# ryogrid/anime-illust-image-searcher

Hardware: AMD Instinct MI355X
Metric: images/sec tagged (ViT fwd) (higher is better)
Workload: dtype f16; 1 GPU; wd-tagger ViT-B/16 448px 16-bit-operand forward + sigmoid + MCut tag selection, batch 64 per GPU, u8 NHWC images resident in HBM (BASELINE.json configs[1]); batch_per_gpu=64, image=448x448x3 u8, classes=10861, parallelism=single GPU

## Files before the change

### anime-illust-image-searcher_amd/csrc/gemm.hip

```cpp
#include <atomic>
#include <cstdlib>
#include <type_traits>

#include "vit_internal.h"

namespace hipts {
namespace {

#ifndef HIPTS_DW_SNAKE
#define HIPTS_DW_SNAKE 1
#endif
#if HIPTS_DW_SNAKE
#define HIPTS_SNAKE_J(i, j) (((i) & 1) ? 3 - (j) : (j))
#else
#define HIPTS_SNAKE_J(i, j) (j)
#endif
#ifndef HIPTS_MFMA_ORDER
#define HIPTS_MFMA_ORDER 1
#endif
#include "gemm_epi.h"


template <int EPI>
__global__ __launch_bounds__(512) void gemm_kernel(const GemmArgs a, int tiles_m, int tiles_n) {
    extern __shared__ __attribute__((aligned(16))) char smem[];
    const int tid = threadIdx.x, lane = tid & 63, wave = tid >> 6;
    const int wave_m = wave >> 2, wave_n = wave & 3;

    const int nwg = tiles_m * tiles_n;
    int bid = blockIdx.x;
    {
        const int q = nwg >> 3, r = nwg & 7, xcd = bid & 7, loc = bid >> 3;
        bid = (xcd < r ? xcd * (q + 1) : r * (q + 1) + (xcd - r) * q) + loc;
    }
    const int tm = bid / tiles_n, tn = bid % tiles_n;
    const int m0 = tm * BM, n0 = tn * BN;
    const int K = a.K, nt = K / BK;
    const int w_rows = tiles_n * BN;

    f32x4 acc[8][4];
#pragma unroll
    for (int i = 0; i < 8; ++i)
#pragma unroll
        for (int j = 0; j < 4; ++j) acc[i][j] = f32x4{0.f, 0.f, 0.f, 0.f};

    stage_tile(a.A, a.M, K, m0, 0, smem, wave, lane);
    stage_tile(a.W, w_rows, K, n0, 0, smem + TILE_BYTES, wave, lane);
    asm volatile("s_waitcnt vmcnt(0)" ::: "memory");
    __syncthreads();

    for (int t = 0; t < nt; ++t) {
        char* cur = smem + (t & 1) * STAGE_BYTES;
        if (t + 1 < nt) {
            char* nxt = smem + ((t + 1) & 1) * STAGE_BYTES;
            stage_tile(a.A, a.M, K, m0, t + 1, nxt, wave, lane);
            stage_tile(a.W, w_rows, K, n0, t + 1, nxt + TILE_BYTES, wave, lane);
        }
#pragma unroll
        for (int kk = 0; kk < 2; ++kk) {
            bf16x8 af[8], wf[4];
#pragma unroll
            for (int j = 0; j < 4; ++j) wf[j] = read_frag(cur + TILE_BYTES, wave_n * 4 + j, kk, lane);
#pragma unroll
            for (int i = 0; i < 8; ++i) af[i] = read_frag(cur, wave_m * 8 + i, kk, lane);
#pragma unroll
            for (int i = 0; i < 8; ++i)
#pragma unroll
                for (int j = 0; j < 4; ++j) {
                    if constexpr (EPI == EPI_VT)
                        acc[i][j] = __builtin_amdgcn_mfma_f32_16x16x32_bf16(af[i], wf[j], acc[i][j], 0, 0, 0);
                    else
                        acc[i][j] = __builtin_amdgcn_mfma_f32_16x16x32_bf16(wf[j], af[i], acc[i][j], 0, 0, 0);
                }
        }
        asm volatile("s_waitcnt vmcnt(0)" ::: "memory");
        __syncthreads();
    }

    gemm_epilogue<EPI>(a, acc, m0, n0, wave_m, wave_n, lane);
}

__device__ __forceinline__ void wait_vmcnt(int n) {
    switch (n) {
        case 0: asm volatile("s_waitcnt vmcnt(0)" ::: "memory"); break;
        case 1: asm volatile("s_waitcnt vmcnt(1)" ::: "memory"); break;
        case 2: asm volatile("s_waitcnt vmcnt(2)" ::: "memory"); break;
        case 3: asm volatile("s_waitcnt vmcnt(3)" ::: "memory"); break;
        case 4: asm volatile("s_waitcnt vmcnt(4)" ::: "memory"); break;
        case 5: asm volatile("s_waitcnt vmcnt(5)" ::: "memory"); break;
        case 6: asm volatile("s_waitcnt vmcnt(6)" ::: "memory"); break;
        case 7: asm volatile("s_waitcnt vmcnt(7)" ::: "memory"); break;
        default: asm volatile("s_waitcnt vmcnt(8)" ::: "memory"); break;
    }
}

template <int EPI, int MR = 8, bool F16 = false, bool OP8 = false, bool SK = false, bool INT = false>
__global__ __launch_bounds__(512) __attribute__((amdgpu_num_vgpr(HIPTS_INT_DEPTH == 3 ? 256 : 240))) void gemm_pp_kernel(const GemmArgs a, int tiles_m, int tiles_n) {
    static_assert(!INT || (EPI == EPI_RESID_XG && MR == 8 && !OP8 && !SK), "INT: the residual epilogue's interior form");
    static_assert(!OP8 || (F16 && MR == 8), "e4m3 operands: half 16-bit outputs, full tiles");
    static_assert(!SK || (!OP8 && MR == 8), "split-K: 16-bit operands, full tiles");
    constexpr int TBM = 2 * MR * 16;
    extern __shared__ __attribute__((aligned(16))) char smem[];
    __shared__ float2 st_table[256];
    __shared__ float2 sw_red[EPI == EPI_SWIGLU ? 1024 : 1];
    __shared__ unsigned sk_ticket[SK ? 4 : 1];
    __shared__ f32x4 colvec[INT ? (EPI == EPI_RESID_XGI ? 768 : 512) : 1];
    const int tid = threadIdx.x, lane = tid & 63;
    const int wave = __builtin_amdgcn_readfirstlane(tid >> 6);
    const int wave_m = wave >> 2, wave_n = wave & 3;

    const int nwg = tiles_m * tiles_n;
    auto tile_origin = [&](int id, int& m0, int& n0) {
        const int q = nwg >> 3, r = nwg & 7, xcd = id & 7, loc = id >> 3;
        const int bid = (xcd < r ? xcd * (q + 1) : r * (q + 1) + (xcd - r) * q) + loc;
        if (a.raster_gn > 0) {
            const int per = tiles_m * a.raster_gn, grp = bid / per, rem = bid - grp * per;
            const int left = tiles_n - grp * a.raster_gn, gn = left < a.raster_gn ? left : a.raster_gn;
            m0 = (rem / gn) * TBM;
            n0 = (grp * a.raster_gn + rem % gn) * BN;
            return;
        }
        if (a.raster_gm > 0) {
            const int per = a.raster_gm * tiles_n, grp = bid / per, rem = bid - grp * per;
            const int left = tiles_m - grp * a.raster_gm, gm = left < a.raster_gm ? left : a.raster_gm;
            m0 = (grp * a.raster_gm + rem % gm) * TBM;
            n0 = (rem / gm) * BN;
            return;
        }
        m0 = (bid / tiles_n) * TBM;
        n0 = (bid % tiles_n) * BN;
    };
    const int K = OP8 ? a.K / 2 : a.K, nt_all = K / BK;
    const int w_rows = tiles_n * BN;
    const int S = SK ? a.sk_slices : 1;
    const int n_items = SK ? a.sk_first + (nwg - a.sk_first) * S : nwg;
    auto decode = [&](int item, int& tid_, int& slice_, int& kt0_, int& ntl_) {
        if (!SK || item < a.sk_first) {
            tid_ = item; slice_ = -1; kt0_ = 0; ntl_ = nt_all;
        } else {
            const int j = item - a.sk_first;
            tid_ = a.sk_first + j / S;
            slice_ = j - (j / S) * S;
            kt0_ = slice_ * nt_all / S;
            ntl_ = (slice_ + 1) * nt_all / S - kt0_;
        }
    };
    const int scale_w = (127 - a.w_exp) * 0x01010101, scale_1 = 127 * 0x01010101;

    int stamp_tile = 0;
#define PPSTAMP(idx)                                                                                     \
    do {                                                                                                 \
        if (a.stamps && blockIdx.x == 8 && stamp_tile < 8) {                                             \
            __builtin_amdgcn_sched_barrier(0);                                                           \
            const unsigned long long ts_ = __builtin_readcyclecounter();                                 \
            if (lane == 0) a.stamps[wave * 64 + stamp_tile * 8 + (idx)] = ts_;                           \
            __builtin_amdgcn_sched_barrier(0);                                                           \
        }                                                                                                \
    } while (0)
    int tile = blockIdx.x, m0, n0;
    int tix, slice, kt0, nt;
    decode(tile, tix, slice, kt0, nt);
    tile_origin(tix, m0, n0);
    int par = 0;

    if (wave * 4 < 4 * MR) stage_tile(a.A, a.M, K, m0, kt0, smem, wave, lane);
    stage_tile(a.W, w_rows, K, n0, kt0, smem + TILE_BYTES, wave, lane);
    if constexpr (INT) {
        for (int i = tid; i < (a.N >> 2); i += 512) {
            colvec[i] = reinterpret_cast<const f32x4*>(a.ln_gamma)[i];
            colvec[256 + i] = reinterpret_cast<const f32x4*>(a.bias)[i];
            if constexpr (EPI == EPI_RESID_XGI) colvec[512 + i] = reinterpret_cast<const f32x4*>(a.col_u)[i];
        }
        asm volatile("s_waitcnt lgkmcnt(0)" ::: "memory");
    }

    for (;;) {
        f32x4 acc[MR][4];
#pragma unroll
        for (int i = 0; i < MR; ++i)
#pragma unroll
            for (int j = 0; j < 4; ++j) acc[i][j] = f32x4{0.f, 0.f, 0.f, 0.f};

        const bf16_t* src[8];
        int dst[8];
        {
            const int row_in = lane >> 3;
            const int chunk = (lane & 7) ^ row_in;
            auto slot = [&](int idx, bool isW, int rb8) {
                int grow = (isW ? n0 : m0) + rb8 * 8 + row_in;
                const int lim = isW ? w_rows : a.M;
                grow = grow < lim ? grow : lim - 1;
                src[idx] = (isW ? a.W : a.A) + (size_t)grow * K + (size_t)(kt0 + 1) * BK + chunk * 8;
                dst[idx] = (isW ? TILE_BYTES : 0) + rb8 * 1024;
            };
            for (int u = 0; u < 2; ++u) {
                const int e = 2 * wave + u;
                slot(0 + u, true, e);
                slot(2 + u, true, 16 + e);
                slot(4 + u, false, e < 8 ? e : 2 * MR + (e - 8));
            }
            if constexpr (MR == 8) {
                for (int u = 0; u < 2; ++u) {
                    const int e = 2 * wave + u;
                    slot(6 + u, false, e < 8 ? 8 + e : 2 * MR + 8 + (e - 8));
                }
            } else if constexpr (MR == 6) {
                slot(6, false, wave < 4 ? 8 + wave : 2 * MR + 8 + (wave - 4));
                src[7] = src[6];
                dst[7] = dst[6];
            } else {
                static_assert(MR == 7, "tile heights: 256, 224 or 192 rows");
                auto hi = [](int f) { return f < 6 ? 8 + f : 2 * MR + 8 + (f - 6); };
                if (wave < 4) {
                    slot(6, false, hi(2 * wave));
                    slot(7, false, hi(2 * wave + 1));
                } else {
                    slot(6, false, hi(8 + (wave - 4)));
                    src[7] = src[6];
                    dst[7] = dst[6];
                }
            }
        }
        const int n_hi = (MR == 8 || (MR == 7 && wave < 4)) ? 2 : 1;
        PPSTAMP(0);
        asm volatile("s_waitcnt vmcnt(0)" ::: "memory");
        PPSTAMP(1);
        __builtin_amdgcn_s_barrier();
        if (wave_m == 1) __builtin_amdgcn_s_barrier();
        PPSTAMP(2);
        if (a.stamps && blockIdx.x == 8 && stamp_tile < 8 && lane == 0) a.stamps[wave * 64 + stamp_tile * 8 + 6] = wall_clock64();
        if (HIPTS_STAGE_AHEAD && !HIPTS_STAGE_ORDER_OLD && nt > 1) {
            char* st1 = smem + ((par + 1) & 1) * STAGE_BYTES;
            for (int k : {4, 5, 0, 1}) {
                glds16(src[k], st1 + dst[k]);
                src[k] += BK;
            }
        }

        bf16x8 wf[2][4];
        i32x8 wf8[4], af8[4];
        unsigned xpf = 0;
        for (int t = 0; t < nt; ++t) {
            const char* cur = smem + ((par + t) & 1) * STAGE_BYTES;
            char* nxt = smem + ((par + t + 1) & 1) * STAGE_BYTES;
            const bool more = t + 1 < nt;
#pragma unroll
            for (int p = 0; p < 4; ++p) {
                const int mh = p >> 1, kk = p & 1;
                bf16x8 af[4];
                if constexpr (OP8) {
                    if (p < 2) {
#pragma unroll
                        for (int jj = 0; jj < 2; ++jj) wf8[2 * kk + jj] = read_frag8(cur + TILE_BYTES, wave_n * 4 + 2 * kk + jj, lane);
                    }
                    if (kk == 0) {
#pragma unroll
                        for (int i = 0; i < 4; ++i) af8[i] = read_frag8(cur, wave_m * MR + mh * 4 + i, lane);
                    }
                } else {
                if (p < 2) {
#pragma unroll
                    for (int j = 0; j < 4; ++j) wf[kk][j] = read_frag(cur + TILE_BYTES, wave_n * 4 + j, kk, lane);
                }
#pragma unroll
                for (int i = 0; i < 4; ++i)
                    if (mh * 4 + i < MR) af[i] = read_frag(cur, wave_m * MR + mh * 4 + i, kk, lane);
                }
                if (more) {
                    auto issue = [&](int k) {
                        glds16(src[k], nxt + dst[k]);
                        src[k] += BK;
                    };
                    if (HIPTS_STAGE_ORDER_OLD) {
                        issue(2 * p);
                        if (p < 3 || n_hi == 2) issue(2 * p + 1);
                        if (p == 3) {
                            if (n_hi == 2) asm volatile("s_waitcnt vmcnt(2)" ::: "memory");
                            else asm volatile("s_waitcnt vmcnt(1)" ::: "memory");
                        } else if (p == 1) {
                            asm volatile("s_waitcnt vmcnt(4)" ::: "memory");
                        }
                    } else if (HIPTS_STAGE_AHEAD) {
                        if (p == 0) {
                            issue(2); issue(3);
                        } else if (p == 1) {
                            issue(6);
                            if (n_hi == 2) issue(7);
                            wait_vmcnt(6 + n_hi);
                        } else if (p == 3) {
                            if (t + 2 < nt) {
                                for (int k : {4, 5, 0, 1}) {
                                    glds16(src[k], const_cast<char*>(cur) + dst[k]);
                                    src[k] += BK;
                                }
                                wait_vmcnt(n_hi + 4);
                            } else {
                                wait_vmcnt(n_hi);
                            }
                        }
                    } else {
                        if (p == 0) {
                            issue(4); issue(5); issue(0); issue(1);
                            if (HIPTS_STAGE_W_EARLY) { issue(2); issue(3); }
                        } else if (p == 1) {
                            if (!HIPTS_STAGE_W_EARLY) { issue(2); issue(3); }
                            asm volatile("s_waitcnt vmcnt(6)" ::: "memory");
                        } else if (p == 2) {
                            issue(6);
                            if (n_hi == 2) issue(7);
                        } else {
                            if (n_hi == 2) asm volatile("s_waitcnt vmcnt(2)" ::: "memory");
                            else asm volatile("s_waitcnt vmcnt(1)" ::: "memory");
                        }
                    }
                } else if (p == 1) {
                    asm volatile("s_waitcnt vmcnt(0)" ::: "memory");
                }
                if constexpr (INT) {
                    if (!more && p == 2 && a.epi_prefetch) {
                        const int ldx = a.ld_out ? a.ld_out : a.N;
                        const char* xb = reinterpret_cast<const char*>(a.out_f32 + (size_t)(m0 + wave_m * 128) * ldx + n0 + wave_n * 64);
                        const unsigned o0 = (unsigned)(((lane >> 1) * ldx + (lane & 1) * 32) * 4), ost = (unsigned)(32 * ldx * 4);
                        asm volatile("global_load_dword %0, %1, %5\n\tglobal_load_dword %0, %2, %5\n\tglobal_load_dword %0, %3, %5\n\tglobal_load_dword %0, %4, %5"
                                     : "=&v"(xpf)
                                     : "v"(o0), "v"(o0 + ost), "v"(o0 + 2 * ost), "v"(o0 + 3 * ost), "s"(xb)
                                     : "memory");
                    }
                }
                __builtin_amdgcn_sched_barrier(0);
                __builtin_amdgcn_s_barrier();
                __builtin_amdgcn_sched_barrier(0);
                asm volatile("s_waitcnt lgkmcnt(0)" ::: "memory");
                __builtin_amdgcn_sched_barrier(0);
                __builtin_amdgcn_s_setprio(1);
                if constexpr (OP8) {
#pragma unroll
                    for (int i = 0; i < 4; ++i)
#pragma unroll
                        for (int jj = 0; jj < 2; ++jj) {
                            const int j = 2 * kk + jj;
                            if constexpr (EPI == EPI_VT)
                                acc[mh * 4 + i][j] = mfma_16x16x128_e4m3(af8[i], wf8[j], acc[mh * 4 + i][j], scale_1, scale_w);
                            else
                                acc[mh * 4 + i][j] = mfma_16x16x128_e4m3(wf8[j], af8[i], acc[mh * 4 + i][j], scale_w, scale_1);
                        }
                } else {
#pragma unroll
                for (int ij = 0; ij < 16; ++ij) {
#if HIPTS_MFMA_ORDER == 2
                    const int j = ij >> 2, i = ij & 3;
#elif HIPTS_MFMA_ORDER == 1
                    const int i = ij >> 2, j = (i & 1) ? 3 - (ij & 3) : (ij & 3);
#else
                    const int i = ij >> 2, j = ij & 3;
#endif
                    if (mh * 4 + i >= MR) continue;
                    if constexpr (EPI == EPI_VT)
                        acc[mh * 4 + i][j] = mfma_16x16x32<F16>(af[i], wf[kk][j], acc[mh * 4 + i][j]);
                    else
                        acc[mh * 4 + i][j] = mfma_16x16x32<F16>(wf[kk][j], af[i], acc[mh * 4 + i][j]);
                }
                }
                __builtin_amdgcn_s_setprio(0);
                __builtin_amdgcn_sched_barrier(0);
                __builtin_amdgcn_s_barrier();
                __builtin_amdgcn_sched_barrier(0);
            }
        }
        if (wave_m == 0) __builtin_amdgcn_s_barrier();
        PPSTAMP(3);
        if (a.stamps && blockIdx.x == 8 && stamp_tile < 8 && lane == 0) a.stamps[wave * 64 + stamp_tile * 8 + 7] = wall_clock64();

        f32x4 bias_pre[4];
        if constexpr (INT) {
#pragma unroll
            for (int j = 0; j < 4; ++j) bias_pre[j] = f32x4{0.f, 0.f, 0.f, 0.f};
        } else {
            load_bias<EPI>(a, n0, wave_n, lane, bias_pre);
        }
        constexpr bool FOLDABLE = EPI == EPI_VT || EPI == EPI_GELU || EPI == EPI_STAR || EPI == EPI_QK || EPI == EPI_QK_ROPE || EPI == EPI_SWIGLU ||
                                  EPI == EPI_RESID_ROWSTAT || EPI == EPI_RESID_XGI;
        const bool fold_st = FOLDABLE && a.stat_in != nullptr;
        const bool fold_many = fold_st && a.stat_in_blocks > 4;
        float2 st_pv[4];
        if (fold_st && !fold_many && tid < TBM) row_stat_request(a, m0 + tid, st_pv);
        const int next = tile + gridDim.x;
        const bool has_next = next < n_items;
        int m0n = 0, n0n = 0, tixn = 0, slicen = -1, kt0n = 0, ntn = nt_all;
        const int par_next = (par + nt) & 1;
        if (has_next) {
            decode(next, tixn, slicen, kt0n, ntn);
            tile_origin(tixn, m0n, n0n);
            char* st = smem + par_next * STAGE_BYTES;
            if (wave * 4 < 4 * MR) stage_tile(a.A, a.M, K, m0n, kt0n, st, wave, lane);
            stage_tile(a.W, w_rows, K, n0n, kt0n, st + TILE_BYTES, wave, lane);
        }
        PPSTAMP(4);
        bool run_epilogue = true;
        if constexpr (SK) {
            if (slice >= 0) {
                constexpr size_t SLAB = (size_t)TBM * BN * 4;
                const int tl = tix - a.sk_first;
                unsigned* tickets = reinterpret_cast<unsigned*>(a.sk_ws);
                char* slabs = reinterpret_cast<char*>(a.sk_ws) + 4096 + (size_t)tl * S * SLAB;
                {
                    const auto rs = __builtin_amdgcn_make_buffer_rsrc(slabs + (size_t)slice * SLAB, 0, (int)SLAB, 0x00020000);
                    typedef unsigned int u32x4 __attribute__((ext_vector_type(4)));
#pragma unroll
                    for (int i = 0; i < MR; ++i)
#pragma unroll
                        for (int j = 0; j < 4; ++j)
                            __builtin_amdgcn_raw_buffer_store_b128(__builtin_bit_cast(u32x4, acc[i][j]), rs, (((wave * MR + i) * 4 + j) * 64 + lane) * 16, 0, 16);
                }
                asm volatile("s_waitcnt vmcnt(0)" ::: "memory");
                __builtin_amdgcn_s_barrier();
                if (threadIdx.x == 0)
                    sk_ticket[0] = __hip_atomic_fetch_add(tickets + tl, 1u, __ATOMIC_RELAXED, __HIP_MEMORY_SCOPE_AGENT);
                __builtin_amdgcn_fence(__ATOMIC_RELEASE, "workgroup");
                __builtin_amdgcn_s_barrier();
                __builtin_amdgcn_fence(__ATOMIC_ACQUIRE, "workgroup");
                const unsigned ticket = sk_ticket[0];
                if (ticket != (unsigned)(S - 1)) {
                    run_epilogue = false;
                } else {
                    if (threadIdx.x == 0) {
                        __builtin_amdgcn_fence(__ATOMIC_ACQUIRE, "agent");
                        __hip_atomic_store(tickets + tl, 0u, __ATOMIC_RELAXED, __HIP_MEMORY_SCOPE_AGENT);
                    }
                    asm volatile("s_waitcnt vmcnt(0)" ::: "memory");
                    __builtin_amdgcn_s_barrier();
                    const f32x4* sl = reinterpret_cast<const f32x4*>(slabs) + (size_t)(wave * MR * 4) * 64 + lane;
#pragma unroll
                    for (int i = 0; i < MR; ++i) {
#pragma unroll
                        for (int j = 0; j < 4; ++j) acc[i][j] = sl[(size_t)(i * 4 + j) * 64];
                        for (int sx = 1; sx < S; ++sx) {
                            const f32x4* sp = sl + (size_t)sx * (SLAB / 16);
                            f32x4 v[4];
#pragma unroll
                            for (int j = 0; j < 4; ++j) v[j] = sp[(size_t)(i * 4 + j) * 64];
#pragma unroll
                            for (int j = 0; j < 4; ++j) acc[i][j] = acc[i][j] + v[j];
                        }
                    }
                }
            }
        }
        if (run_epilogue) {
        if (fold_st) {
            if (fold_many) {
                if (tid < TBM) st_table[tid] = row_stat(a, m0 + tid);
            } else if (tid < TBM) st_table[tid] = row_stat_finish(a, st_pv);
            __builtin_amdgcn_fence(__ATOMIC_RELEASE, "workgroup");
            __builtin_amdgcn_s_barrier();
            __builtin_amdgcn_fence(__ATOMIC_ACQUIRE, "workgroup");
        }
        bool staged = false;
        if constexpr (EPI == EPI_VT || EPI == EPI_GELU || EPI == EPI_STAR || EPI == EPI_QK || EPI == EPI_QK_ROPE || EPI == EPI_SWIGLU) {
            const bool ok = EPI == EPI_VT                            ? (a.tokens % 8 == 0 && a.tokens_pad % 8 == 0)
                            : (EPI == EPI_QK || EPI == EPI_QK_ROPE) ? (a.dim % 64 == 0)
                                                                     : ((a.ld_out ? a.ld_out : a.N) % 8 == 0);
            if (ok) {
                float2* red = (EPI == EPI_SWIGLU && a.stat_part) ? sw_red : nullptr;
                gemm_epilogue_staged<EPI, MR, F16>(a, acc, m0, n0, wave_m, wave_n, lane,
                                                   smem + ((par + nt + 1) & 1) * STAGE_BYTES + wave * 8192, bias_pre, fold_st ? st_table : nullptr, red);
                staged = true;
                if constexpr (EPI == EPI_SWIGLU) {
                    if (red) {
                        __builtin_amdgcn_fence(__ATOMIC_RELEASE, "workgroup");
                        __builtin_amdgcn_s_barrier();
                        __builtin_amdgcn_fence(__ATOMIC_ACQUIRE, "workgroup");
                        if (tid < TBM) {
                            const float2 p0 = red[tid * 4], p1 = red[tid * 4 + 1], p2 = red[tid * 4 + 2], p3 = red[tid * 4 + 3];
                            const int m = m0 + tid;
                            if (m < a.M)
                                *reinterpret_cast<float2*>(a.stat_part + 2 * ((size_t)(n0 >> 8) * a.stat_stride + m)) =
                                    make_float2((p0.x + p1.x) + (p2.x + p3.x), (p0.y + p1.y) + (p2.y + p3.y));
                        }
                    }
                }
            }
        }
        if (!staged)
            gemm_epilogue<EPI, MR, F16, INT>(a, acc, m0, n0, wave_m, wave_n, lane, bias_pre, smem + ((par + nt + 1) & 1) * STAGE_BYTES,
                                             fold_st ? st_table : nullptr, INT ? colvec : nullptr);
        }
        if (a.epi_prio) __builtin_amdgcn_s_setprio(0);
        if constexpr (INT) asm volatile("" ::"v"(xpf));
        PPSTAMP(5);
        ++stamp_tile;
        if (!has_next) break;
        tile = next;
        tix = tixn;
        slice = slicen;
        kt0 = kt0n;
        nt = ntn;
        m0 = m0n;
        n0 = n0n;
        par = par_next;
    }
}

#define PP2_STAMP(idx)                                                                                   \
    if constexpr (STAMP) {                                                                               \
        if (blockIdx.x == 0 && (t == 10 || t == 11)) {                                                   \
            __builtin_amdgcn_sched_barrier(0);                                                           \
            unsigned long long ts_;                                                                      \
            asm volatile("s_memtime %0\n\ts_waitcnt lgkmcnt(0)" : "=s"(ts_)::"memory");                 \
            if (lane == 0) a.stamps[wave * 64 + (t - 10) * 16 + mh * 8 + (idx)] = ts_;                   \
            __builtin_amdgcn_sched_barrier(0);                                                           \
        }                                                                                                \
    }

template <int EPI, bool STAMP = false>
__global__ __launch_bounds__(512) void gemm_pp2_kernel(const GemmArgs a, int tiles_m, int tiles_n) {
    extern __shared__ __attribute__((aligned(16))) char smem[];
    const int tid = threadIdx.x, lane = tid & 63;
    const int wave = __builtin_amdgcn_readfirstlane(tid >> 6);
    const int wave_m = wave >> 2, wave_n = wave & 3;

    const int nwg = tiles_m * tiles_n;
    int bid = blockIdx.x;
    {
        const int q = nwg >> 3, r = nwg & 7, xcd = bid & 7, loc = bid >> 3;
        bid = (xcd < r ? xcd * (q + 1) : r * (q + 1) + (xcd - r) * q) + loc;
    }
    const int tm = bid / tiles_n, tn = bid % tiles_n;
    const int m0 = tm * BM, n0 = tn * BN;
    const int K = a.K, nt = K / BK;
    const int w_rows = tiles_n * BN;

    f32x4 acc[8][4];
#pragma unroll
    for (int i = 0; i < 8; ++i)
#pragma unroll
        for (int j = 0; j < 4; ++j) acc[i][j] = f32x4{0.f, 0.f, 0.f, 0.f};

    stage_tile(a.A, a.M, K, m0, 0, smem, wave, lane);
    stage_tile(a.W, w_rows, K, n0, 0, smem + TILE_BYTES, wave, lane);

    const bf16_t* src[8];
    int dst[8];
    {
        const int row_in = lane >> 3;
        const int chunk = (lane & 7) ^ row_in;
        auto slot = [&](int idx, bool isW, int rb8) {
            int grow = (isW ? n0 : m0) + rb8 * 8 + row_in;
            const int lim = isW ? w_rows : a.M;
            grow = grow < lim ? grow : lim - 1;
            src[idx] = (isW ? a.W : a.A) + (size_t)grow * K + BK + chunk * 8;
            dst[idx] = (isW ? TILE_BYTES : 0) + rb8 * 1024;
        };
        for (int u = 0; u < 4; ++u) slot(u, true, 4 * wave + u);
        for (int u = 0; u < 2; ++u) {
            const int e = 2 * wave + u;
            slot(4 + u, false, e < 8 ? e : e + 8);
            slot(6 + u, false, e < 8 ? 8 + e : 16 + e);
        }
    }
    asm volatile("s_waitcnt vmcnt(0)" ::: "memory");
    __builtin_amdgcn_s_barrier();
    if (wave_m == 1) __builtin_amdgcn_s_barrier();

    bf16x8 wf[2][4];
    for (int t = 0; t < nt; ++t) {
        const char* cur = smem + (t & 1) * STAGE_BYTES;
        char* nxt = smem + ((t + 1) & 1) * STAGE_BYTES;
        const bool more = t + 1 < nt;
#pragma unroll
        for (int mh = 0; mh < 2; ++mh) {
            PP2_STAMP(0)
            bf16x8 af[2][4];
            if (mh == 0) {
#pragma unroll
                for (int kk = 0; kk < 2; ++kk)
#pragma unroll
                    for (int j = 0; j < 4; ++j) wf[kk][j] = read_frag(cur + TILE_BYTES, wave_n * 4 + j, kk, lane);
            }
#pragma unroll
            for (int kk = 0; kk < 2; ++kk)
#pragma unroll
                for (int i = 0; i < 4; ++i) af[kk][i] = read_frag(cur, wave_m * 8 + mh * 4 + i, kk, lane);
            if (more) {
                if (mh == 0) {
#pragma unroll
                    for (int u = 0; u < 6; ++u) {
                        glds16(src[u], nxt + dst[u]);
                        src[u] += BK;
                    }
                    PP2_STAMP(1)
                    asm volatile("s_waitcnt vmcnt(6)" ::: "memory");
                } else {
#pragma unroll
                    for (int u = 6; u < 8; ++u) {
                        glds16(src[u], nxt + dst[u]);
                        src[u] += BK;
                    }
                    PP2_STAMP(1)
                    asm volatile("s_waitcnt vmcnt(2)" ::: "memory");
                }
            } else if (mh == 0) {
                asm volatile("s_waitcnt vmcnt(0)" ::: "memory");
            }
            PP2_STAMP(2)
            __builtin_amdgcn_sched_barrier(0);
            __builtin_amdgcn_s_barrier();
            __builtin_amdgcn_sched_barrier(0);
            PP2_STAMP(3)
            asm volatile("s_waitcnt lgkmcnt(0)" ::: "memory");
            __builtin_amdgcn_sched_barrier(0);
            PP2_STAMP(4)
            __builtin_amdgcn_s_setprio(1);
#pragma unroll
            for (int kk = 0; kk < 2; ++kk)
#pragma unroll
                for (int i = 0; i < 4; ++i)
#pragma unroll
                    for (int j = 0; j < 4; ++j) {
                        if constexpr (EPI == EPI_VT)
                            acc[mh * 4 + i][j] = __builtin_amdgcn_mfma_f32_16x16x32_bf16(af[kk][i], wf[kk][j], acc[mh * 4 + i][j], 0, 0, 0);
                        else
                            acc[mh * 4 + i][j] = __builtin_amdgcn_mfma_f32_16x16x32_bf16(wf[kk][j], af[kk][i], acc[mh * 4 + i][j], 0, 0, 0);
                    }
            __builtin_amdgcn_s_setprio(0);
            PP2_STAMP(5)
            __builtin_amdgcn_sched_barrier(0);
            __builtin_amdgcn_s_barrier();
            __builtin_amdgcn_sched_barrier(0);
            PP2_STAMP(6)
        }
    }
    if (wave_m == 0) __builtin_amdgcn_s_barrier();
    gemm_epilogue<EPI>(a, acc, m0, n0, wave_m, wave_n, lane);
}

constexpr int S3_BN = 128, S3_BK = 32, S3_STAGE = (BM + S3_BN) * S3_BK * 2, S3_LDS = 3 * S3_STAGE;

__device__ __forceinline__ void s3_stage(const GemmArgs& a, int m0, int n0, int w_rows, int kt, char* st, int wave, int lane) {
    const int row_in = lane >> 2;
    const int chunk = (lane & 3) ^ (((row_in >> 3) & 1) << 1);
    const size_t koff = (size_t)kt * S3_BK + chunk * 8;
#pragma unroll
    for (int i = 0; i < 4; ++i) {
        const int rb = wave * 4 + i;
        int grow = m0 + rb * 16 + row_in;
        grow = grow < a.M ? grow : a.M - 1;
        glds16(a.A + (size_t)grow * a.K + koff, st + rb * 1024);
    }
#pragma unroll
    for (int i = 0; i < 2; ++i) {
        const int rb = wave * 2 + i;
        int grow = n0 + rb * 16 + row_in;
        grow = grow < w_rows ? grow : w_rows - 1;
        glds16(a.W + (size_t)grow * a.K + koff, st + BM * S3_BK * 2 + rb * 1024);
    }
}

__device__ __forceinline__ bf16x8 s3_frag(const char* base, int rowblk, int lane) {
    const int r = lane & 15;
    const int c = (lane >> 4) ^ (((r >> 3) & 1) << 1);
    return *reinterpret_cast<const bf16x8*>(base + rowblk * 1024 + r * 64 + c * 16);
}

template <int EPI>
__global__ __launch_bounds__(256, 2) void gemm_s3_kernel(const GemmArgs a, int tiles_m, int tiles_n) {
    extern __shared__ __attribute__((aligned(16))) char smem[];
    const int tid = threadIdx.x, lane = tid & 63;
    const int wave = __builtin_amdgcn_readfirstlane(tid >> 6);
    const int wave_m = wave >> 1, wave_n = wave & 1;
    const int nwg = tiles_m * tiles_n;
    int bid = blockIdx.x;
    {
        const int q = nwg >> 3, r = nwg & 7, xcd = bid & 7, loc = bid >> 3;
        bid = (xcd < r ? xcd * (q + 1) : r * (q + 1) + (xcd - r) * q) + loc;
    }
    const int tm = bid / tiles_n, tn = bid % tiles_n;
    const int m0 = tm * BM, n0 = tn * S3_BN;
    const int nt = a.K / S3_BK;
    const int w_rows = ((a.N + 255) / 256) * 256;

    f32x4 acc[8][4];
#pragma unroll
    for (int i = 0; i < 8; ++i)
#pragma unroll
        for (int j = 0; j < 4; ++j) acc[i][j] = f32x4{0.f, 0.f, 0.f, 0.f};

    s3_stage(a, m0, n0, w_rows, 0, smem, wave, lane);
    if (nt > 1) s3_stage(a, m0, n0, w_rows, 1, smem + S3_STAGE, wave, lane);
    int slot = 0;
    for (int t = 0; t < nt; ++t) {
        if (t + 1 < nt) asm volatile("s_waitcnt vmcnt(6)" ::: "memory");
        else asm volatile("s_waitcnt vmcnt(0)" ::: "memory");
        __builtin_amdgcn_s_barrier();
        __builtin_amdgcn_sched_barrier(0);
        if (t + 2 < nt) {
            int s2 = slot + 2;
            s2 = s2 >= 3 ? s2 - 3 : s2;
            s3_stage(a, m0, n0, w_rows, t + 2, smem + s2 * S3_STAGE, wave, lane);
        }
        const char* cur = smem + slot * S3_STAGE;
        bf16x8 af[8], wf[4];
#pragma unroll
        for (int j = 0; j < 4; ++j) wf[j] = s3_frag(cur + BM * S3_BK * 2, wave_n * 4 + j, lane);
#pragma unroll
        for (int i = 0; i < 8; ++i) af[i] = s3_frag(cur, wave_m * 8 + i, lane);
#pragma unroll
        for (int i = 0; i < 8; ++i)
#pragma unroll
            for (int j = 0; j < 4; ++j) {
                if constexpr (EPI == EPI_VT)
                    acc[i][j] = __builtin_amdgcn_mfma_f32_16x16x32_bf16(af[i], wf[j], acc[i][j], 0, 0, 0);
                else
                    acc[i][j] = __builtin_amdgcn_mfma_f32_16x16x32_bf16(wf[j], af[i], acc[i][j], 0, 0, 0);
            }
        slot = slot == 2 ? 0 : slot + 1;
    }
    gemm_epilogue<EPI>(a, acc, m0, n0, wave_m, wave_n, lane);
}

constexpr int DW_BM = 256, DW_BN = 128, DW_BK = 32;
constexpr int DW_A_BYTES = DW_BM * DW_BK * 2;
constexpr int DW_STAGE = (DW_BM + DW_BN) * DW_BK * 2;
constexpr int DW_LDS = 3 * DW_STAGE;

template <int EPI, bool F16>
__global__ __launch_bounds__(256, 2) void gemm_dw_kernel(const GemmArgs a, int tiles_m, int tiles_n) {
    extern __shared__ __attribute__((aligned(16))) char smem[];
    const int tid = threadIdx.x, lane = tid & 63;
    const int wave = __builtin_amdgcn_readfirstlane(tid >> 6);
    const int wave_m = wave >> 1, wave_n = wave & 1;
    const int nwg = tiles_m * tiles_n;
    int bid = blockIdx.x;
    {
        const int q = nwg >> 3, r = nwg & 7, xcd = bid & 7, loc = bid >> 3;
        bid = (xcd < r ? xcd * (q + 1) : r * (q + 1) + (xcd - r) * q) + loc;
    }
    const int tm = bid / tiles_n, tn = bid % tiles_n;
    const int m0 = tm * DW_BM, n0 = tn * DW_BN;
    const int K = a.K, nt = K / DW_BK;
    const int w_rows = ((a.N + 255) / 256) * 256;

    const bf16_t* src[6];
    int dst[6];
    {
        const int r = lane >> 2, q = (lane & 3) ^ ((r >> 2) & 3);
#pragma unroll
        for (int i = 0; i < 4; ++i) {
            const int rb = wave * 4 + i;
            int grow = m0 + rb * 16 + r;
            grow = grow < a.M ? grow : a.M - 1;
            src[i] = a.A + (size_t)grow * K + q * 8;
            dst[i] = rb * 1024;
        }
#pragma unroll
        for (int i = 0; i < 2; ++i) {
            const int rb = wave * 2 + i;
            int grow = n0 + rb * 16 + r;
            grow = grow < w_rows ? grow : w_rows - 1;
            src[4 + i] = a.W + (size_t)grow * K + q * 8;
            dst[4 + i] = DW_A_BYTES + rb * 1024;
        }
    }
    const int frag_off = (lane & 15) * 64 + (((lane >> 4) ^ (((lane & 15) >> 2) & 3)) * 16);
    auto issue = [&](int i, char* st) {
        glds16(src[i], st + dst[i]);
        src[i] += DW_BK;
    };
    auto frag = [&](const char* base, int rb) { return *reinterpret_cast<const bf16x8*>(base + rb * 1024 + frag_off); };

    f32x4 acc[8][4];
#pragma unroll
    for (int i = 0; i < 8; ++i)
#pragma unroll
        for (int j = 0; j < 4; ++j) acc[i][j] = f32x4{0.f, 0.f, 0.f, 0.f};

    const bool trace = a.stamps && a.trace && blockIdx.x < 4096;
    if (trace && tid == 0) {
        a.stamps[blockIdx.x * 8 + 0] = __builtin_amdgcn_s_getreg(63492);
        a.stamps[blockIdx.x * 8 + 1] = __builtin_amdgcn_s_getreg(63508);
        a.stamps[blockIdx.x * 8 + 2] = wall_clock64();
    }
    const int npro = nt < 3 ? nt : 3;
    for (int s0 = 0; s0 < npro; ++s0)
#pragma unroll
        for (int i = 0; i < 6; ++i) issue(i, smem + s0 * DW_STAGE);
    if (npro == 3) asm volatile("s_waitcnt vmcnt(12)" ::: "memory");
    else if (npro == 2) asm volatile("s_waitcnt vmcnt(6)" ::: "memory");
    else asm volatile("s_waitcnt vmcnt(0)" ::: "memory");
    __builtin_amdgcn_s_barrier();
    __builtin_amdgcn_sched_barrier(0);

    bf16x8 wfr[2][4], alo[2][4], ahi[4];
#pragma unroll
    for (int j = 0; j < 4; ++j) wfr[0][j] = frag(smem + DW_A_BYTES, wave_n * 4 + j);
#pragma unroll
    for (int i = 0; i < 4; ++i) alo[0][i] = frag(smem, wave_m * 8 + i);

    int slot = 0;
    unsigned long long wait_cyc = 0, bar_cyc = 0;
    const unsigned long long loop_t0 = a.stamps ? __builtin_readcyclecounter() : 0;
    const unsigned long long wall_t0 = a.stamps ? wall_clock64() : 0;
    auto mm = [&](f32x4& c, const bf16x8& av, const bf16x8& wv) {
        if constexpr (EPI == EPI_VT) c = mfma_16x16x32<F16>(av, wv, c);
        else c = mfma_16x16x32<F16>(wv, av, c);
    };
    auto step = [&](auto H1, auto H2, auto H3, auto U) {
        constexpr bool has1 = decltype(H1)::value, has2 = decltype(H2)::value, has3 = decltype(H3)::value;
        constexpr int u = decltype(U)::value;
        const char* cur = smem + slot * DW_STAGE;
        const int slot1 = slot == 2 ? 0 : slot + 1;
        const char* nx = smem + slot1 * DW_STAGE;
#pragma unroll
        for (int i = 0; i < 4; ++i)
#pragma unroll
            for (int j = 0; j < 4; ++j) {
                mm(acc[i][HIPTS_SNAKE_J(i, j)], alo[u][i], wfr[u][HIPTS_SNAKE_J(i, j)]);
                if (i == 0) ahi[j] = frag(cur, wave_m * 8 + 4 + j);
                __builtin_amdgcn_sched_barrier(0);
            }
        if constexpr (has1) {
            unsigned long long q0 = 0, q1 = 0;
            if (a.stamps) q0 = __builtin_readcyclecounter();
            if constexpr (has2) asm volatile("s_waitcnt vmcnt(6) lgkmcnt(0)" ::: "memory");
            else asm volatile("s_waitcnt vmcnt(0) lgkmcnt(0)" ::: "memory");
            if (a.stamps) q1 = __builtin_readcyclecounter();
            __builtin_amdgcn_s_barrier();
            if (a.stamps) { const unsigned long long q2 = __builtin_readcyclecounter(); wait_cyc += q1 - q0; bar_cyc += q2 - q1; }
        }
        __builtin_amdgcn_sched_barrier(0);
        char* fill = smem + slot * DW_STAGE;
#pragma unroll
        for (int i = 0; i < 4; ++i)
#pragma unroll
            for (int j = 0; j < 4; ++j) {
                mm(acc[4 + i][HIPTS_SNAKE_J(i, j)], ahi[i], wfr[u][HIPTS_SNAKE_J(i, j)]);
                const int idx = i * 4 + j;
                if constexpr (has1) {
                    if (idx < 4) wfr[u ^ 1][idx] = frag(nx + DW_A_BYTES, wave_n * 4 + idx);
                    else if (idx < 8) alo[u ^ 1][idx - 4] = frag(nx, wave_m * 8 + (idx - 4));
                }
                if constexpr (has3) {
                    if (idx >= 8 && idx < 14) issue(idx - 8, fill);
                }
                __builtin_amdgcn_sched_barrier(0);
            }
        slot = slot1;
    };
    using T = std::true_type;
    using F = std::false_type;
    using U0 = std::integral_constant<int, 0>;
    using U1 = std::integral_constant<int, 1>;
    for (int s = 0; s + 6 <= nt; s += 2) {
        step(T{}, T{}, T{}, U0{});
        step(T{}, T{}, T{}, U1{});
    }
    if (nt >= 4) {
        step(T{}, T{}, T{}, U0{});
        step(T{}, T{}, F{}, U1{});
    }
    step(T{}, F{}, F{}, U0{});
    step(F{}, F{}, F{}, U1{});
    if (trace && tid == 0) a.stamps[blockIdx.x * 8 + 3] = wall_clock64();
    if (a.stamps && !trace && blockIdx.x == 8 && lane == 0) {
        a.stamps[wave * 64 + 0] = __builtin_readcyclecounter() - loop_t0;
        a.stamps[wave * 64 + 1] = wait_cyc;
        a.stamps[wave * 64 + 2] = bar_cyc;
        a.stamps[wave * 64 + 3] = wall_clock64() - wall_t0;
    }
    __builtin_amdgcn_s_barrier();
    if constexpr (EPI == EPI_VT || EPI == EPI_GELU || EPI == EPI_STAR || EPI == EPI_QK || EPI == EPI_QK_ROPE || EPI == EPI_SWIGLU) {
        const bool ok = EPI == EPI_VT                            ? (a.tokens % 8 == 0 && a.tokens_pad % 8 == 0)
                        : (EPI == EPI_QK || EPI == EPI_QK_ROPE) ? (a.dim % 64 == 0)
                                                                 : ((a.ld_out ? a.ld_out : a.N) % 8 == 0);
        if (ok) {
            const float2* st_tab = nullptr;
            if (a.stat_in) {
                float2 pv[4];
                row_stat_request(a, m0 + tid, pv);
                float2* tab = reinterpret_cast<float2*>(smem + 4 * 8192 * 2);
                tab[tid] = row_stat_finish(a, pv);
                __builtin_amdgcn_fence(__ATOMIC_RELEASE, "workgroup");
                __builtin_amdgcn_s_barrier();
                __builtin_amdgcn_fence(__ATOMIC_ACQUIRE, "workgroup");
                st_tab = tab;
            }
            gemm_epilogue_staged<EPI, 8, F16>(a, acc, m0, n0, wave_m, wave_n, lane, smem + wave * 8192, nullptr, st_tab);
            if (trace && tid == 0) a.stamps[blockIdx.x * 8 + 4] = wall_clock64();
            return;
        }
    }
    gemm_epilogue<EPI, 8, F16>(a, acc, m0, n0, wave_m, wave_n, lane, nullptr, smem);
    if (trace && tid == 0) a.stamps[blockIdx.x * 8 + 4] = wall_clock64();
}

std::atomic<long long> g_q4_mask{-1};
unsigned gemm_q4_mask() {
    long long v = g_q4_mask.load(std::memory_order_relaxed);
    if (v < 0) {
        v = getenv("HIPTS_GEMM_Q4") ? (long long)(unsigned)strtoul(getenv("HIPTS_GEMM_Q4"), nullptr, 0) : (long long)GEMM_Q4_DEFAULT_MASK;
        g_q4_mask.store(v, std::memory_order_relaxed);
    }
    return (unsigned)v;
}

int gemm_variant() {
    static int v = -1;
    if (v < 0) {
        const char* e = getenv("HIPTS_GEMM");
        v = (e && strcmp(e, "v1") == 0) ? 0 : (e && strcmp(e, "pp2") == 0) ? 3 : (e && strcmp(e, "s3") == 0) ? 2 : (e && strcmp(e, "dw") == 0) ? 4 : 1;
    }
    return v;
}

template <int EPI>
int launch_t(const GemmArgs& a, hipStream_t s) {
    int dev = 0;
    const int cus_dev = current_device_cus(&dev);
    static PerDevice attr;
    {
      std::lock_guard<std::mutex> lk(attr.mu);
      if (!attr.done(dev)) {
        HIPTS_HIP(hipFuncSetAttribute((const void*)gemm_kernel<EPI>, hipFuncAttributeMaxDynamicSharedMemorySize, LDS_BYTES));
        HIPTS_HIP(hipFuncSetAttribute((const void*)gemm_pp_kernel<EPI, 8, false>, hipFuncAttributeMaxDynamicSharedMemorySize, LDS_BYTES));
        HIPTS_HIP(hipFuncSetAttribute((const void*)gemm_pp_kernel<EPI, 7, false>, hipFuncAttributeMaxDynamicSharedMemorySize, LDS_BYTES));
        HIPTS_HIP(hipFuncSetAttribute((const void*)gemm_pp_kernel<EPI, 8, true>, hipFuncAttributeMaxDynamicSharedMemorySize, LDS_BYTES));
        HIPTS_HIP(hipFuncSetAttribute((const void*)gemm_pp_kernel<EPI, 7, true>, hipFuncAttributeMaxDynamicSharedMemorySize, LDS_BYTES));
        HIPTS_HIP(hipFuncSetAttribute((const void*)gemm_pp_kernel<EPI, 6, true>, hipFuncAttributeMaxDynamicSharedMemorySize, LDS_BYTES));
        HIPTS_HIP(hipFuncSetAttribute((const void*)gemm_pp2_kernel<EPI, false>, hipFuncAttributeMaxDynamicSharedMemorySize, LDS_BYTES));
        HIPTS_HIP(hipFuncSetAttribute((const void*)gemm_s3_kernel<EPI>, hipFuncAttributeMaxDynamicSharedMemorySize, S3_LDS));
        HIPTS_HIP(hipFuncSetAttribute((const void*)gemm_dw_kernel<EPI, false>, hipFuncAttributeMaxDynamicSharedMemorySize, DW_LDS));
        HIPTS_HIP(hipFuncSetAttribute((const void*)gemm_dw_kernel<EPI, true>, hipFuncAttributeMaxDynamicSharedMemorySize, DW_LDS));
        attr.mark(dev);
      }
    }
    const int tiles_m = (a.M + BM - 1) / BM;
    if (a.op8) {
        if constexpr (EPI == EPI_STAR || EPI == EPI_RESID || EPI == EPI_RESCALE || EPI == EPI_RESID_LN || EPI == EPI_QK || EPI == EPI_VT ||
                      EPI == EPI_BIAS) {
            static PerDevice attr8;
            {
                std::lock_guard<std::mutex> lk(attr8.mu);
                if (!attr8.done(dev)) {
                    HIPTS_HIP(hipFuncSetAttribute((const void*)gemm_pp_kernel<EPI, 8, true, true>, hipFuncAttributeMaxDynamicSharedMemorySize, LDS_BYTES));
                    attr8.mark(dev);
                }
            }
            const int cus8 = cus_dev;
            const int tiles_n = (a.N + BN - 1) / BN;
            const int ntile = tiles_m * tiles_n;
            const int slots = cus8 >= 8 ? cus8 / 8 * 8 : cus8;
            gemm_pp_kernel<EPI, 8, true, true><<<ntile > slots ? slots : ntile, 512, LDS_BYTES, s>>>(a, tiles_m, tiles_n);
            HIPTS_LAUNCH_CHECK();
            return HIPTS_OK;
        } else {
            return set_error(HIPTS_ERR_INVALID, "gemm: e4m3 operands are not built for epilogue %d", (int)EPI);
        }
    }
    int variant = gemm_variant();
    if (EPI == EPI_QK_ROPE || EPI == EPI_SWIGLU || EPI == EPI_RESID_XG || EPI == EPI_RESID_XGI) variant = 1;
    if (EPI == EPI_RESID_LN) variant = 1;
    if (variant == 1 && EPI != EPI_HEAD && EPI != EPI_RESID_LN && (!getenv("HIPTS_GEMM") || EPI == EPI_QK_ROPE || EPI == EPI_SWIGLU || EPI == EPI_RESID_XG || EPI == EPI_RESID_XGI)) {
        const int cus0 = cus_dev;
        static const bool auto_dw = !(getenv("HIPTS_GEMM_AUTO_DW") && atoi(getenv("HIPTS_GEMM_AUTO_DW")) == 0);
        static const int dw_limit4 = getenv("HIPTS_GEMM_DW_LIMIT") ? atoi(getenv("HIPTS_GEMM_DW_LIMIT")) : 2;
        if (auto_dw && (long)tiles_m * ((a.N + BN - 1) / BN) * 4 <= (long)cus0 * dw_limit4 && a.M > BM && !((EPI == EPI_RESID_XG || EPI == EPI_RESID_XGI || EPI == EPI_SWIGLU) && a.stat_part)) variant = 4;
    }
    {
        static const unsigned dw_mask = getenv("HIPTS_GEMM_DW_MASK") ? (unsigned)strtoul(getenv("HIPTS_GEMM_DW_MASK"), nullptr, 0) : 0u;
#ifdef HIPTS_X_DW_STAT
        if (variant == 1 && ((dw_mask >> (int)EPI) & 1u) && a.M > BM) variant = 4;
#else
        if (variant == 1 && ((dw_mask >> (int)EPI) & 1u) && a.M > BM && !((EPI == EPI_RESID_XG || EPI == EPI_RESID_XGI) && a.stat_part)) variant = 4;
#endif
    }
    HIPTS_REQUIRE(!a.f16 || variant == 1 || variant == 4, "half-precision operands are only built for the pp and dw GEMM loops");
    if (variant == 4) {
        const int tiles_n = (a.N + DW_BN - 1) / DW_BN;
        if (a.f16) gemm_dw_kernel<EPI, true><<<tiles_m * tiles_n, 256, DW_LDS, s>>>(a, tiles_m, tiles_n);
        else gemm_dw_kernel<EPI, false><<<tiles_m * tiles_n, 256, DW_LDS, s>>>(a, tiles_m, tiles_n);
    } else if (variant == 2) {
        const int tiles_n = (a.N + S3_BN - 1) / S3_BN;
        gemm_s3_kernel<EPI><<<tiles_m * tiles_n, 256, S3_LDS, s>>>(a, tiles_m, tiles_n);
    } else {
        const int tiles_n = (a.N + BN - 1) / BN;
        if (variant == 3) {
            if constexpr (EPI == EPI_GELU) {
                if (a.stamps) {
                    HIPTS_HIP(hipFuncSetAttribute((const void*)gemm_pp2_kernel<EPI, true>, hipFuncAttributeMaxDynamicSharedMemorySize, LDS_BYTES));
                    gemm_pp2_kernel<EPI, true><<<tiles_m * tiles_n, 512, LDS_BYTES, s>>>(a, tiles_m, tiles_n);
                    HIPTS_LAUNCH_CHECK();
                    return HIPTS_OK;
                }
            }
            gemm_pp2_kernel<EPI><<<tiles_m * tiles_n, 512, LDS_BYTES, s>>>(a, tiles_m, tiles_n);
        }
        else if (variant == 1) {
            const int cus = cus_dev;
            static const int min_mr = !getenv("HIPTS_GEMM_BM") ? 6 : strcmp(getenv("HIPTS_GEMM_BM"), "256") == 0 ? 8 : strcmp(getenv("HIPTS_GEMM_BM"), "224") == 0 ? 7 : 6;
            auto tiles_of = [&](int mr) { return (a.M + 32 * mr - 1) / (32 * mr); };
            auto cost_of = [&](int mr) { return ((long)tiles_of(mr) * tiles_n + cus - 1) / cus * (32 * mr); };
            int mr = 8;
            static const int mr_shared = getenv("HIPTS_GEMM_MR_SHARED") ? atoi(getenv("HIPTS_GEMM_MR_SHARED")) : -1;
            if (!a.shared_chip || mr_shared == 1 || (mr_shared != 0 && (long)tiles_of(8) * tiles_n < cus)) {
                long best = cost_of(8) * 93;
                for (int c = 7; c >= (a.f16 ? min_mr : (min_mr > 7 ? min_mr : 7)); --c)
                    if (cost_of(c) * 100 < best) {
                        best = cost_of(c) * 100;
                        mr = c;
                    }
            }
            if (EPI == EPI_HEAD && a.sk_ws && getenv("HIPTS_GEMM_SPLITK_HEAD") && atoi(getenv("HIPTS_GEMM_SPLITK_HEAD")) >= 2) mr = 8;
            const int tiles_mr = tiles_of(mr);
            static const bool persist = !(getenv("HIPTS_GEMM_PERSIST") && strcmp(getenv("HIPTS_GEMM_PERSIST"), "0") == 0);
            const int ntile = tiles_mr * tiles_n;
            const int slots = cus >= 8 ? cus / 8 * 8 : cus;
            const int grid = (persist && ntile > slots) ? slots : ntile;
            static const int raster = getenv("HIPTS_GEMM_RASTER") ? atoi(getenv("HIPTS_GEMM_RASTER")) : 8;
            static const int raster_gn = getenv("HIPTS_GEMM_RASTER_GN") ? atoi(getenv("HIPTS_GEMM_RASTER_GN")) : 6;
            GemmArgs ar = a;
            static const int epi_prio = getenv("HIPTS_EPI_PRIO") ? atoi(getenv("HIPTS_EPI_PRIO")) : 0;
            ar.epi_prio = epi_prio;
            static const int epi_prefetch = getenv("HIPTS_EPI_PREFETCH") ? atoi(getenv("HIPTS_EPI_PREFETCH")) : 0;
            ar.epi_prefetch = epi_prefetch;
            ar.raster_gm = (raster > 0 && tiles_n >= 8) ? raster : 0;
            ar.raster_gn = (raster_gn > 0 && tiles_n >= 8 && tiles_n > raster_gn) ? raster_gn : 0;
            {
                const unsigned q4_mask = gemm_q4_mask();
                if (mr == 8 && ((q4_mask >> (int)EPI) & 1u)) {
                    bool handled = false;
                    const int st = launch_gemm_q4((GemmEpilogue)EPI, ar, s, &handled);
                    if (handled) return st;
                }
            }
            static const bool resid_general = getenv("HIPTS_RESID_GENERAL") && atoi(getenv("HIPTS_RESID_GENERAL")) != 0;
            if constexpr (EPI == EPI_RESID || EPI == EPI_RESID_XG || EPI == EPI_RESID_XGI || EPI == EPI_RESID_ROWSTAT || EPI == EPI_HEAD) {
                static const int sk_env = getenv("HIPTS_GEMM_SPLITK") ? atoi(getenv("HIPTS_GEMM_SPLITK")) : 0;
                static const int sk_head = getenv("HIPTS_GEMM_SPLITK_HEAD") ? atoi(getenv("HIPTS_GEMM_SPLITK_HEAD")) : 0;
                const int sk_max = EPI == EPI_HEAD ? (tiles_mr == 1 ? sk_head : 0) : sk_env;
                static const int sk_minkt = getenv("HIPTS_GEMM_SPLITK_MINKT") ? atoi(getenv("HIPTS_GEMM_SPLITK_MINKT")) : 5;
                const int nkt = a.K / BK;
                const int rem = ntile % slots;
                if (a.sk_ws && mr == 8 && sk_max >= 2 && rem > 0 && rem * 2 <= slots && rem <= 1024) {
                    int sl = std::min(sk_max, std::min(slots / rem, nkt / (sk_minkt > 0 ? sk_minkt : 1)));
                    while (sl >= 2 && 4096 + (size_t)rem * sl * ((size_t)BM * BN * 4) > a.sk_ws_bytes) --sl;
                    if (sl >= 2) {
                        static PerDevice attr_sk;
                        {
                            std::lock_guard<std::mutex> lk(attr_sk.mu);
                            if (!attr_sk.done(dev)) {
                                HIPTS_HIP(hipFuncSetAttribute((const void*)gemm_pp_kernel<EPI, 8, false, false, true>, hipFuncAttributeMaxDynamicSharedMemorySize, LDS_BYTES));
                                HIPTS_HIP(hipFuncSetAttribute((const void*)gemm_pp_kernel<EPI, 8, true, false, true>, hipFuncAttributeMaxDynamicSharedMemorySize, LDS_BYTES));
                                attr_sk.mark(dev);
                            }
                        }
                        ar.sk_first = ntile - rem;
                        ar.sk_slices = sl;
                        const int items = ar.sk_first + rem * sl;
                        const int grid_sk = (persist && items > slots) ? slots : items;
                        if (a.f16) gemm_pp_kernel<EPI, 8, true, false, true><<<grid_sk, 512, LDS_BYTES, s>>>(ar, tiles_m, tiles_n);
                        else gemm_pp_kernel<EPI, 8, false, false, true><<<grid_sk, 512, LDS_BYTES, s>>>(ar, tiles_m, tiles_n);
                        HIPTS_LAUNCH_CHECK();
                        return HIPTS_OK;
                    }
                }
            }
            if constexpr (EPI == EPI_RESID_XG) {
                if (mr == 8 && a.M % 256 == 0 && a.N % 256 == 0 && a.N <= 1024 && !a.pos && !a.res_scale && a.out_bf16 && a.stat_part && !resid_general) {
                    static PerDevice attr_int;
                    {
                        std::lock_guard<std::mutex> lk(attr_int.mu);
                        if (!attr_int.done(dev)) {
                            HIPTS_HIP(hipFuncSetAttribute((const void*)gemm_pp_kernel<EPI, 8, false, false, false, true>, hipFuncAttributeMaxDynamicSharedMemorySize, LDS_BYTES));
                            HIPTS_HIP(hipFuncSetAttribute((const void*)gemm_pp_kernel<EPI, 8, true, false, false, true>, hipFuncAttributeMaxDynamicSharedMemorySize, LDS_BYTES));
                            attr_int.mark(dev);
                        }
                    }
                    if (a.f16) gemm_pp_kernel<EPI, 8, true, false, false, true><<<grid, 512, LDS_BYTES, s>>>(ar, tiles_m, tiles_n);
                    else gemm_pp_kernel<EPI, 8, false, false, false, true><<<grid, 512, LDS_BYTES, s>>>(ar, tiles_m, tiles_n);
                    HIPTS_LAUNCH_CHECK();
                    return HIPTS_OK;
                }
            }
            if (a.f16) {
                if (mr == 6) gemm_pp_kernel<EPI, 6, true><<<grid, 512, LDS_BYTES, s>>>(ar, tiles_mr, tiles_n);
                else if (mr == 7) gemm_pp_kernel<EPI, 7, true><<<grid, 512, LDS_BYTES, s>>>(ar, tiles_mr, tiles_n);
                else gemm_pp_kernel<EPI, 8, true><<<grid, 512, LDS_BYTES, s>>>(ar, tiles_m, tiles_n);
            } else {
                if (mr == 7) gemm_pp_kernel<EPI, 7, false><<<grid, 512, LDS_BYTES, s>>>(ar, tiles_mr, tiles_n);
                else gemm_pp_kernel<EPI, 8, false><<<grid, 512, LDS_BYTES, s>>>(ar, tiles_m, tiles_n);
            }
        }
        else
            gemm_kernel<EPI><<<tiles_m * tiles_n, 512, LDS_BYTES, s>>>(a, tiles_m, tiles_n);
    }
    HIPTS_LAUNCH_CHECK();
    return HIPTS_OK;
}

}

int launch_gemm(GemmEpilogue epi, const GemmArgs& a, hipStream_t s) {
    if (a.op8) HIPTS_REQUIRE(a.K % 128 == 0 && a.K >= 128, "gemm: K=%d must be a positive multiple of 128 with e4m3 operands", a.K);
    if (a.out8)
        HIPTS_REQUIRE((epi == EPI_STAR || epi == EPI_RESID_LN) && (a.ld_out ? a.ld_out : a.N) % 16 == 0,
                      "gemm: e4m3 output needs the STAR / RESID_LN epilogue and a row stride that is a multiple of 16");
    HIPTS_REQUIRE(a.K % BK == 0 && a.K >= BK, "gemm: K=%d must be a positive multiple of %d", a.K, BK);
    HIPTS_REQUIRE(a.M >= 1 && a.N >= 1, "gemm: empty problem");
    if (epi != EPI_HEAD) HIPTS_REQUIRE(a.N % 16 == 0, "gemm: N=%d must be a multiple of 16", a.N);
    if (epi == EPI_VT) HIPTS_REQUIRE(a.M % 4 == 0 && a.tokens % 4 == 0, "gemm: V^T epilogue needs tokens %% 4 == 0");
    if (epi == EPI_QK || epi == EPI_VT) HIPTS_REQUIRE(a.hd_log2 == 5 || a.hd_log2 == 6, "gemm: head_dim must be 32 or 64");
    if (epi == EPI_QK || epi == EPI_QK_ROPE)
        HIPTS_REQUIRE(a.out_bf16 && a.out2_bf16 && a.dim > 0 && a.N <= 3 * a.dim && (a.N <= 2 * a.dim || a.out3_bf16), "gemm: q / k / v outputs missing for N = %d, dim = %d", a.N, a.dim);
    if (epi == EPI_QK_ROPE)
        HIPTS_REQUIRE(a.hd_log2 == 6 && a.dim % 64 == 0 && a.rope && a.rope_tokens >= 0 && a.tokens >= 1, "gemm: QK_ROPE needs head_dim 64 and the rotary table");
    if (epi == EPI_RESID_XG) HIPTS_REQUIRE(!a.rowstat && !a.stat_in, "gemm: RESID_XG ignores an input fold; use RESID_XGI");
    if (epi == EPI_RESID_XGI) HIPTS_REQUIRE((a.rowstat || a.stat_in) && a.col_u, "gemm: RESID_XGI needs rowstat / stat_in and col_u");
    if (epi == EPI_RESID_XG || epi == EPI_RESID_XGI)
        HIPTS_REQUIRE(a.out_f32 && (!a.out_bf16 || (a.ln_gamma && a.N % 8 == 0 && (!a.stat_part || a.stat_stride >= a.M))),
                      "gemm: RESID_XG needs the fp32 stream, col_u with rowstat, and gamma (N %% 8 == 0) with the 16-bit copy");
    if (a.stat_in) HIPTS_REQUIRE(a.stat_in_blocks <= 64 && a.stat_in_blocks >= 1 && a.stat_in_stride >= a.M && a.ln_dim >= 1, "gemm: stat_in needs its block count (<= 64), stride and ln_dim");
    if ((a.rowstat || a.stat_in) && epi != EPI_RESID_ROWSTAT && epi != EPI_RESID_XGI)
        HIPTS_REQUIRE(a.col_u && (epi == EPI_QK || epi == EPI_QK_ROPE || epi == EPI_VT || epi == EPI_GELU || epi == EPI_SWIGLU || epi == EPI_STAR),
                      "gemm: a folded LayerNorm (rowstat) is built for the QK, QK_ROPE, VT, GELU, STAR and SWIGLU epilogues");
    if ((a.rowstat || a.stat_in) && epi != EPI_RESID_ROWSTAT && epi != EPI_RESID_XGI) {
        const int ldo = a.ld_out ? a.ld_out : (epi == EPI_SWIGLU ? a.N / 2 : a.N);
        const bool staged = (epi == EPI_QK || epi == EPI_QK_ROPE) ? a.dim % 64 == 0
                            : epi == EPI_VT                       ? (a.tokens % 8 == 0 && a.tokens_pad % 8 == 0)
                                                                  : ldo % 8 == 0;
        HIPTS_REQUIRE(staged && (gemm_variant() == 1 || gemm_variant() == 4), "gemm: a folded LayerNorm needs the staged epilogue (pp / dw loops, aligned outputs)");
    }
    if (epi == EPI_RESID_ROWSTAT) HIPTS_REQUIRE((a.rowstat || a.stat_in) && a.col_u && a.out_f32, "gemm: RESID_ROWSTAT needs rowstat / stat_in, col_u and the fp32 stream");
    if (epi == EPI_SWIGLU) HIPTS_REQUIRE(!a.stat_part || a.stat_stride >= a.M, "gemm: SWIGLU stat_stride must cover M rows");
    if (epi == EPI_SWIGLU)
        HIPTS_REQUIRE(a.N % 64 == 0 && (a.ld_out ? a.ld_out : a.N / 2) % 8 == 0 && a.out_bf16, "gemm: SWIGLU needs N %% 64 == 0 and an output stride that is a multiple of 8");
    if (epi == EPI_RESCALE) HIPTS_REQUIRE(a.res_scale != nullptr, "gemm: RESCALE epilogue needs res_scale");
    if (epi == EPI_RESID_LS) HIPTS_REQUIRE(a.res_scale && a.out_f32 && !a.x_blocked, "gemm: RESID_LS needs the layer scale and the row-major fp32 stream");
    if (epi == EPI_RESID_LN)
        HIPTS_REQUIRE(a.N <= BN && a.ln_gamma && a.out_bf16 && a.out_f32, "gemm: RESID_LN needs the whole row in one tile (N <= %d), gamma and both outputs", BN);
    switch (epi) {
        case EPI_PATCH: return launch_t<EPI_PATCH>(a, s);
        case EPI_QK: return launch_t<EPI_QK>(a, s);
        case EPI_VT: return launch_t<EPI_VT>(a, s);
        case EPI_RESID: return launch_t<EPI_RESID>(a, s);
        case EPI_GELU: return launch_t<EPI_GELU>(a, s);
        case EPI_HEAD: return launch_t<EPI_HEAD>(a, s);
        case EPI_STAR: return launch_t<EPI_STAR>(a, s);
        case EPI_RESCALE: return launch_t<EPI_RESCALE>(a, s);
        case EPI_BIAS: return launch_t<EPI_BIAS>(a, s);
        case EPI_RESID_LN: return launch_t<EPI_RESID_LN>(a, s);
        case EPI_QK_ROPE: return launch_t<EPI_QK_ROPE>(a, s);
        case EPI_SWIGLU: return launch_t<EPI_SWIGLU>(a, s);
        case EPI_RESID_ROWSTAT: return launch_t<EPI_RESID_ROWSTAT>(a, s);
        case EPI_RESID_XG: return launch_t<EPI_RESID_XG>(a, s);
        case EPI_RESID_XGI: return launch_t<EPI_RESID_XGI>(a, s);
        case EPI_RESID_LS: return launch_t<EPI_RESID_LS>(a, s);
    }
    return set_error(HIPTS_ERR_INVALID, "gemm: unknown epilogue");
}

void set_gemm_q4_mask(unsigned mask) { g_q4_mask.store((long long)mask, std::memory_order_relaxed); }

namespace {
__global__ void gelu_probe_kernel(const f32x4* __restrict__ x, f32x4* __restrict__ y, int n4, int tanh_form) {
    const int i = blockIdx.x * blockDim.x + threadIdx.x;
    if (i < n4) y[i] = gelu_f4(x[i], tanh_form);
}
}

}

extern "C" int hiptsdbg_gelu(const float* x_host, int n, int tanh_form, float* y_host) {
    using namespace hipts;
    HIPTS_TRY(use_device(0));
    HIPTS_REQUIRE(x_host && y_host && n > 0 && n % 4 == 0, "hiptsdbg_gelu: n must be a positive multiple of 4");
    DevBuf x, y;
    HIPTS_TRY(x.alloc((size_t)n * 4));
    HIPTS_TRY(y.alloc((size_t)n * 4));
    HIPTS_TRY(upload(x.p, x_host, (size_t)n * 4));
    gelu_probe_kernel<<<(n / 4 + 255) / 256, 256>>>(x.as<f32x4>(), y.as<f32x4>(), n / 4, tanh_form);
    HIPTS_LAUNCH_CHECK();
    HIPTS_HIP(hipMemcpy(y_host, y.p, (size_t)n * 4, hipMemcpyDeviceToHost));
    return HIPTS_OK;
}
```

### anime-illust-image-searcher_amd/csrc/gemm_epi.h

```cpp

constexpr int BM = 256, BN = 256, BK = 64;
#ifndef HIPTS_STAGE_AHEAD
#define HIPTS_STAGE_AHEAD 1
#endif
#ifndef HIPTS_STAGE_W_EARLY
#define HIPTS_STAGE_W_EARLY 0
#endif
#ifndef HIPTS_STAGE_ORDER_OLD
#define HIPTS_STAGE_ORDER_OLD 0
#endif
#ifndef HIPTS_STAGED_INTERIOR
#define HIPTS_STAGED_INTERIOR 1
#endif
#ifndef HIPTS_INT_DEPTH
#define HIPTS_INT_DEPTH 2
#endif
constexpr int TILE_BYTES = BM * BK * 2;
constexpr int STAGE_BYTES = 2 * TILE_BYTES;
constexpr int LDS_BYTES = 2 * STAGE_BYTES;

__device__ __forceinline__ void glds16(const void* g, void* lds) {
    __builtin_amdgcn_global_load_lds((const __attribute__((address_space(1))) void*)g,
                                     (__attribute__((address_space(3))) void*)lds, 16, 0, 0);
}
// ... 178 lines not shown
#pragma unroll
            for (int r8 = 0; r8 < 8; ++r8) *reinterpret_cast<uint4*>(base + (size_t)r8 * 8 * ld) = v[r8];
        } else {
#pragma unroll
            for (int r8 = 0; r8 < 8; ++r8) {
                const int row = r8 * 8 + lrow;
                const int m = mrow0 + pass * 64 + row;
                const uint4 v = *reinterpret_cast<const uint4*>(region + row * 128 + ((lc ^ ((row >> 1) & 7)) * 16));
                if (pass * 64 + row >= MR * 16 || m >= M || !nvl) continue;
                *reinterpret_cast<uint4*>(out + (size_t)m * ld + ncol0 + lc * 8) = v;
            }
        }
        __builtin_amdgcn_fence(__ATOMIC_ACQUIRE, "wavefront");
    }
}

template <int MR, typename ValueOf>
__device__ __forceinline__ void staged_store_rows8(char* region, int lane, int mrow0, int M, uint8_t* out, int ld, int ncol0, int N,
                                                   ValueOf value_of) {
    const int lr = lane & 15, lq = lane >> 4, lc = lane & 3, lrow = lane >> 2;
    const bool nvl = ncol0 + lc * 16 < N;
#pragma unroll
    for (int pass = 0; pass < 2; ++pass) {
        if (pass) __builtin_amdgcn_wave_barrier();
#pragma unroll
        for (int ii = 0; ii < 4; ++ii) {
            const int i = pass * 4 + ii;
            if (i >= MR) continue;
#pragma unroll
            for (int j = 0; j < 4; ++j) {
                const int row = ii * 16 + lr;
                const int pc = j ^ ((row >> 2) & 3);
                const f32x4 v = value_of(i, j);
                *reinterpret_cast<uint32_t*>(region + row * 64 + pc * 16 + lq * 4) = pack4_e4m3(v[0], v[1], v[2], v[3]);
            }
        }
        __builtin_amdgcn_fence(__ATOMIC_RELEASE, "wavefront");
        __builtin_amdgcn_wave_barrier();
#pragma unroll
        for (int r16 = 0; r16 < 4; ++r16) {
            const int row = r16 * 16 + lrow;
            const int m = mrow0 + pass * 64 + row;
            const uint4 v = *reinterpret_cast<const uint4*>(region + row * 64 + ((lc ^ ((row >> 2) & 3)) * 16));
            if (pass * 64 + row >= MR * 16 || m >= M || !nvl) continue;
            *reinterpret_cast<uint4*>(out + (size_t)m * ld + ncol0 + lc * 16) = v;
        }
        __builtin_amdgcn_fence(__ATOMIC_ACQUIRE, "wavefront");
    }
}

template <bool F16, typename ValueOf>
__device__ __forceinline__ void staged_store_2blocks(char* image, int lane, int mrow_first, int nblk, int M, bf16_t* out, int ld, int ncol0, int N,
                                                     ValueOf value_of) {
    const int lr = lane & 15, lq = lane >> 4, lc = lane & 7, lrow = lane >> 3;
    const bool nvl = ncol0 + lc * 8 < N;
#pragma unroll
    for (int u = 0; u < 2; ++u) {
        if (u >= nblk) continue;
#pragma unroll
        for (int j = 0; j < 4; ++j) {
            const int row = u * 16 + lr;
            const int pc = (j * 2 + (lq >> 1)) ^ ((row >> 1) & 7);
            const f32x4 v = value_of(u, j);
            *reinterpret_cast<bf16x4*>(image + row * 128 + pc * 16 + (lq & 1) * 8) = pack4<F16>(v[0], v[1], v[2], v[3]);
        }
    }
    __builtin_amdgcn_fence(__ATOMIC_RELEASE, "wavefront");
    __builtin_amdgcn_wave_barrier();
#pragma unroll
    for (int r8 = 0; r8 < 4; ++r8) {
        const int row = r8 * 8 + lrow;
        const int m = mrow_first + row;
        const uint4 v = *reinterpret_cast<const uint4*>(image + row * 128 + ((lc ^ ((row >> 1) & 7)) * 16));
        if (row < nblk * 16 && m < M && nvl) *reinterpret_cast<uint4*>(out + (size_t)m * ld + ncol0 + lc * 8) = v;
    }
    __builtin_amdgcn_fence(__ATOMIC_ACQUIRE, "wavefront");
    __builtin_amdgcn_wave_barrier();
}

template <bool F16, typename ValueOf>
__device__ __forceinline__ void staged_store_2blocks_interior(char* image, int lane, bf16_t* out_rows, int ld, ValueOf value_of) {
    const int lr = lane & 15, lq = lane >> 4, lc = lane & 7, lrow = lane >> 3;
#pragma unroll
    for (int u = 0; u < 2; ++u)
#pragma unroll
        for (int j = 0; j < 4; ++j) {
            const int row = u * 16 + lr;
            const int pc = (j * 2 + (lq >> 1)) ^ ((row >> 1) & 7);
            const f32x4 v = value_of(u, j);
            *reinterpret_cast<bf16x4*>(image + row * 128 + pc * 16 + (lq & 1) * 8) = pack4<F16>(v[0], v[1], v[2], v[3]);
        }
    __builtin_amdgcn_fence(__ATOMIC_RELEASE, "wavefront");
    __builtin_amdgcn_wave_barrier();
#pragma unroll
    for (int r8 = 0; r8 < 4; ++r8) {
        const int row = r8 * 8 + lrow;
        const uint4 v = *reinterpret_cast<const uint4*>(image + row * 128 + ((lc ^ ((row >> 1) & 7)) * 16));
        *reinterpret_cast<uint4*>(out_rows + (size_t)row * ld + lc * 8) = v;
    }
    __builtin_amdgcn_fence(__ATOMIC_ACQUIRE, "wavefront");
    __builtin_amdgcn_wave_barrier();
}

template <int MR, bool F16, typename ValueOf>
__device__ __forceinline__ void staged_store_half_rows(char* region, int lane, int mrow0, int M, bf16_t* out, int ld, int ocol0, int Nout,
                                                       ValueOf value_of) {
    const int lr = lane & 15, lq = lane >> 4, lc = lane & 3, lrow = lane >> 2;
    const bool nvl = ocol0 + lc * 8 < Nout;
#pragma unroll
    for (int pass = 0; pass < 2; ++pass) {
        if (pass) __builtin_amdgcn_wave_barrier();
#pragma unroll
        for (int ii = 0; ii < 4; ++ii) {
            const int i = pass * 4 + ii;
            if (i >= MR) continue;
#pragma unroll
            for (int jj = 0; jj < 2; ++jj) {
                const int row = ii * 16 + lr;
                const int pc = (jj * 2 + (lq >> 1)) ^ ((row >> 2) & 3);
                const f32x4 v = value_of(i, jj);
                *reinterpret_cast<bf16x4*>(region + row * 64 + pc * 16 + (lq & 1) * 8) = pack4<F16>(v[0], v[1], v[2], v[3]);
            }
        }
        __builtin_amdgcn_fence(__ATOMIC_RELEASE, "wavefront");
        __builtin_amdgcn_wave_barrier();
        if (HIPTS_STAGED_INTERIOR && mrow0 + pass * 64 + 64 <= M && pass * 64 + 64 <= MR * 16 && ocol0 + 32 <= Nout) {
            bf16_t* base = out + (size_t)(mrow0 + pass * 64 + lrow) * ld + ocol0 + lc * 8;
            uint4 v[4];
#pragma unroll
            for (int r16 = 0; r16 < 4; ++r16) {
                const int row = r16 * 16 + lrow;
                v[r16] = *reinterpret_cast<const uint4*>(region + row * 64 + ((lc ^ ((row >> 2) & 3)) * 16));
            }
#pragma unroll
            for (int r16 = 0; r16 < 4; ++r16) *reinterpret_cast<uint4*>(base + (size_t)r16 * 16 * ld) = v[r16];
        } else {
#pragma unroll
            for (int r16 = 0; r16 < 4; ++r16) {
                const int row = r16 * 16 + lrow;
                const int m = mrow0 + pass * 64 + row;
                const uint4 v = *reinterpret_cast<const uint4*>(region + row * 64 + ((lc ^ ((row >> 2) & 3)) * 16));
                if (pass * 64 + row >= MR * 16 || m >= M || !nvl) continue;
                *reinterpret_cast<uint4*>(out + (size_t)m * ld + ocol0 + lc * 8) = v;
            }
        }
        __builtin_amdgcn_fence(__ATOMIC_ACQUIRE, "wavefront");
    }
}

template <int EPI, int MR = 8, bool F16 = false, bool INT = false>
__device__ __forceinline__ void gemm_epilogue(const GemmArgs& a, f32x4 (&acc)[MR][4], int m0, int n0, int wave_m, int wave_n,
                                              int lane, const f32x4* bias_pre = nullptr, char* scratch = nullptr, const float2* st_lds = nullptr,
                                              const f32x4* colvec = nullptr, bool finish_stats = true) {
    const int lr = lane & 15, lq = lane >> 4;
    const int ld = a.ld_out ? a.ld_out : a.N;
    f32x4 bias_v[4];
    if (bias_pre) {
#pragma unroll
        for (int j = 0; j < 4; ++j) bias_v[j] = bias_pre[j];
    } else {
        load_bias<EPI>(a, n0, wave_n, lane, bias_v);
    }
    if constexpr (EPI == EPI_VT) {
        float bv[4];
#pragma unroll
        for (int j = 0; j < 4; ++j) bv[j] = bias_v[j][0];
#pragma unroll
        for (int i = 0; i < MR; ++i) {
            const int m = m0 + wave_m * (MR * 16) + i * 16 + 4 * lq;
            if (m >= a.M) continue;
            const int b = m / a.tokens, t = m - b * a.tokens;
#pragma unroll
            for (int j = 0; j < 4; ++j) {
                const int n = n0 + wave_n * 64 + j * 16 + lr;
                if (n >= a.N) continue;
                const f32x4 c = acc[i][j];
                const int head = n >> a.hd_log2, d = n & ((1 << a.hd_log2) - 1);
                const bf16x4 o = pack4<F16>(c[0] + bv[j], c[1] + bv[j], c[2] + bv[j], c[3] + bv[j]);
                *reinterpret_cast<bf16x4*>(a.out_bf16 + ((((size_t)(b * a.heads + head)) << a.hd_log2) + d) * a.tokens_pad + t) = o;
            }
        }
    } else if constexpr (EPI == EPI_HEAD) {
#pragma unroll
        for (int i = 0; i < MR; ++i) {
            const int m = m0 + wave_m * (MR * 16) + i * 16 + lr;
            if (m >= a.M) continue;
#pragma unroll
            for (int j = 0; j < 4; ++j) {
                const int n = n0 + wave_n * 64 + j * 16 + 4 * lq;
#pragma unroll
                for (int e = 0; e < 4; ++e) {
                    if (n + e < a.N) {
                        const float v = acc[i][j][e] + a.bias[n + e];
                        if (a.out_f32) a.out_f32[(size_t)m * ld + n + e] = v;
                        if (a.out2_f32) a.out2_f32[(size_t)m * ld + n + e] = 1.0f / (1.0f + expf(-v));
                    }
                }
            }
        }
    } else {
        int nc[4];
        bool nv[4];
        f32x4 bv[4];
#pragma unroll
        for (int j = 0; j < 4; ++j) {
            nc[j] = n0 + wave_n * 64 + j * 16 + 4 * lq;
            nv[j] = nc[j] < a.N;
            bv[j] = bias_v[j];
        }
        if constexpr (EPI == EPI_RESID_LN) {
            const bool scaled = a.res_scale != nullptr;
            f32x4 rs[4];
#pragma unroll
            for (int j = 0; j < 4; ++j)
                rs[j] = (scaled && nv[j]) ? *reinterpret_cast<const f32x4*>(a.res_scale + nc[j]) : f32x4{1.f, 1.f, 1.f, 1.f};
            constexpr int RB = 2;
#pragma unroll
            for (int i2 = 0; i2 < MR; i2 += RB) {
                f32x4 xv[RB][4];
#pragma unroll
                for (int u = 0; u < RB; ++u) {
                    if (i2 + u >= MR) continue;
                    const int m = m0 + wave_m * (MR * 16) + (i2 + u) * 16 + lr;
                    const int mr = m < a.M ? m : a.M - 1;
#pragma unroll
                    for (int j = 0; j < 4; ++j) xv[u][j] = nv[j] ? *reinterpret_cast<const f32x4*>(a.out_f32 + x_off(a, mr, nc[j], ld)) : f32x4{0.f, 0.f, 0.f, 0.f};
                }
#pragma unroll
                for (int u = 0; u < RB; ++u) {
                    if (i2 + u >= MR) continue;
                    const int m = m0 + wave_m * (MR * 16) + (i2 + u) * 16 + lr;
                    const int mr = m < a.M ? m : a.M - 1;
#pragma unroll
                    for (int j = 0; j < 4; ++j) {
                        acc[i2 + u][j] = nv[j] ? xv[u][j] * rs[j] + (acc[i2 + u][j] + bv[j]) : f32x4{0.f, 0.f, 0.f, 0.f};
                        if (nv[j] && m < a.M) *reinterpret_cast<f32x4*>(a.out_f32 + x_off(a, mr, nc[j], ld)) = acc[i2 + u][j];
                    }
                }
            }
            float* red = reinterpret_cast<float*>(scratch);
            const float inv_n = 1.0f / (float)a.N;
            float mean[MR], rstd[MR];
#pragma unroll
            for (int pass = 0; pass < 2; ++pass) {
#pragma unroll
                for (int i = 0; i < MR; ++i) {
                    float sacc = 0.f;
#pragma unroll
                    for (int j = 0; j < 4; ++j) {
                        if (!nv[j]) continue;
                        if (pass == 0) {
                            sacc += (acc[i][j][0] + acc[i][j][1]) + (acc[i][j][2] + acc[i][j][3]);
                        } else {
                            const f32x4 d = acc[i][j] - mean[i];
                            sacc += (d[0] * d[0] + d[1] * d[1]) + (d[2] * d[2] + d[3] * d[3]);
                        }
                    }
                    sacc += __shfl_xor(sacc, 16);
                    sacc += __shfl_xor(sacc, 32);
                    if (lq == 0) red[(wave_m * (MR * 16) + i * 16 + lr) * 4 + wave_n] = sacc;
                }
                __builtin_amdgcn_fence(__ATOMIC_RELEASE, "workgroup");
                __builtin_amdgcn_s_barrier();
                __builtin_amdgcn_fence(__ATOMIC_ACQUIRE, "workgroup");
#pragma unroll
                for (int i = 0; i < MR; ++i) {
                    const f32x4 p = *reinterpret_cast<const f32x4*>(red + (wave_m * (MR * 16) + i * 16 + lr) * 4);
                    const float t = ((p[0] + p[1]) + (p[2] + p[3])) * inv_n;
                    if (pass == 0) mean[i] = t;
                    else rstd[i] = 1.0f / sqrtf(t + a.ln_eps);
                }
                __builtin_amdgcn_s_barrier();
            }
            f32x4 gv[4], bt[4];
#pragma unroll
            for (int j = 0; j < 4; ++j) {
                gv[j] = nv[j] ? *reinterpret_cast<const f32x4*>(a.ln_gamma + nc[j]) : f32x4{0.f, 0.f, 0.f, 0.f};
                bt[j] = (a.ln_beta && nv[j]) ? *reinterpret_cast<const f32x4*>(a.ln_beta + nc[j]) : f32x4{0.f, 0.f, 0.f, 0.f};
            }
            const int wave_id = wave_m * 4 + wave_n;
            if (a.out8)
                staged_store_rows8<MR>(scratch + wave_id * 8192, lane, m0 + wave_m * (MR * 16), a.M, reinterpret_cast<uint8_t*>(a.out_bf16), ld,
                                       n0 + wave_n * 64, a.N, [&](int i, int j) { return (acc[i][j] - mean[i]) * rstd[i] * gv[j] + bt[j]; });
            else
            staged_store_rows<MR, F16>(scratch + wave_id * 8192, lane, m0 + wave_m * (MR * 16), a.M, a.out_bf16, ld, n0 + wave_n * 64, a.N,
                                       [&](int i, int j) { return (acc[i][j] - mean[i]) * rstd[i] * gv[j] + bt[j]; });
            return;
        }
        if constexpr (EPI == EPI_RESID_XG || EPI == EPI_RESID_XGI) {
            constexpr bool fold = EPI == EPI_RESID_XGI;
            f32x4 uv[4];
#pragma unroll
            for (int j = 0; j < 4; ++j) uv[j] = (!INT && fold && nv[j]) ? *reinterpret_cast<const f32x4*>(a.col_u + nc[j]) : f32x4{0.f, 0.f, 0.f, 0.f};
            constexpr int RB = 2;
            const int ncol0 = n0 + wave_n * 64;
            const bool copy = a.out_bf16 != nullptr;
            f32x4 gv[4];
#pragma unroll
            for (int j = 0; j < 4; ++j)
                gv[j] = (!INT && copy && nv[j]) ? *reinterpret_cast<const f32x4*>(a.ln_gamma + nc[j]) : f32x4{0.f, 0.f, 0.f, 0.f};
            char* image = scratch + (wave_m * 4 + wave_n) * 4096;
            float2* red = reinterpret_cast<float2*>(scratch + 8 * 4096);
            if constexpr (INT) {
                static_assert(MR == 8, "interior epilogue: full tiles");
                const f32x4* cvec = colvec + (ncol0 >> 2);
                const int lane_off = a.x_blocked ? lr * 16 + 4 * lq : lr * ld + 4 * lq;
                const size_t rb_step = a.x_blocked ? (size_t)(ld >> 4) * 256 : (size_t)16 * ld;
                const int cb_step = a.x_blocked ? 256 : 16;
                float* base = a.out_f32 + x_off(a, m0 + wave_m * 128, ncol0, ld);
                constexpr int DEPTH = HIPTS_INT_DEPTH;
                f32x4 xv[DEPTH][RB][4];
                auto request = [&](int buf, int i2) {
#pragma unroll
                    for (int u = 0; u < RB; ++u)
#pragma unroll
                        for (int j = 0; j < 4; ++j)
                            xv[buf][u][j] = *reinterpret_cast<const f32x4*>(base + (size_t)(i2 + u) * rb_step + lane_off + j * cb_step);
                };
                request(0, 0);
                if constexpr (DEPTH == 3) request(1, RB);
#pragma unroll
                for (int i2 = 0; i2 < 8; i2 += RB) {
                    epi_turn(a, wave_m, i2 / RB);
                    const int cur = (i2 / RB) % DEPTH;
                    if constexpr (DEPTH == 3) {
                        if (i2 + 2 * RB < 8) request((cur + 2) % 3, i2 + 2 * RB);
                    } else {
                        if (i2 + RB < 8) request(cur ^ 1, i2 + RB);
                    }
                    __builtin_amdgcn_sched_barrier(0);
#pragma unroll
                    for (int u = 0; u < RB; ++u) {
                        float2 st = make_float2(1.f, 0.f);
                        if constexpr (fold) st = st_lds ? st_lds[wave_m * 128 + (i2 + u) * 16 + lr] : row_stat(a, m0 + wave_m * 128 + (i2 + u) * 16 + lr);
#pragma unroll
                        for (int j = 0; j < 4; ++j) {
                            const f32x4 bj = cvec[256 + j * 4 + lq];
                            if constexpr (fold) acc[i2 + u][j] = xv[cur][u][j] + (acc[i2 + u][j] * st.x + (bj - cvec[512 + j * 4 + lq] * st.y));
                            else acc[i2 + u][j] = xv[cur][u][j] + (acc[i2 + u][j] + bj);
                            *reinterpret_cast<f32x4*>(base + (size_t)(i2 + u) * rb_step + lane_off + j * cb_step) = acc[i2 + u][j];
                        }
                    }
#pragma unroll
                    for (int u = 0; u < RB; ++u) {
                        const int i = i2 + u;
                        f32x4 t = acc[i][0], q = acc[i][0] * acc[i][0];
#pragma unroll
                        for (int j = 1; j < 4; ++j) {
                            t = t + acc[i][j];
                            q = q + acc[i][j] * acc[i][j];
                        }
                        float s1 = (t[0] + t[1]) + (t[2] + t[3]), s2 = (q[0] + q[1]) + (q[2] + q[3]);
                        s1 += __shfl_xor(s1, 16); s2 += __shfl_xor(s2, 16);
                        s1 += __shfl_xor(s1, 32); s2 += __shfl_xor(s2, 32);
                        if (lq == 0) red[(wave_m * 128 + i * 16 + lr) * 4 + wave_n] = make_float2(s1, s2);
                    }
                    staged_store_2blocks_interior<F16>(image, lane, a.out_bf16 + (size_t)(m0 + wave_m * 128 + i2 * 16) * ld + ncol0, ld,
                                                       [&](int u, int j) { return acc[i2 + u][j] * cvec[j * 4 + lq]; });
                    __builtin_amdgcn_sched_barrier(0);
                }
            } else {
#pragma unroll
            for (int i2 = 0; i2 < MR; i2 += RB) {
                epi_turn(a, wave_m, i2 / RB);
                f32x4 xv[RB][4];
                float2 st[RB];
#pragma unroll
                for (int u = 0; u < RB; ++u) {
                    if (i2 + u >= MR) continue;
                    const int m = m0 + wave_m * (MR * 16) + (i2 + u) * 16 + lr;
                    const int mc = m < a.M ? m : a.M - 1;
                    st[u] = fold ? (st_lds ? st_lds[mc - m0] : row_stat(a, mc)) : make_float2(1.f, 0.f);
#pragma unroll
                    for (int j = 0; j < 4; ++j)
                        xv[u][j] = !nv[j] ? f32x4{0.f, 0.f, 0.f, 0.f}
                                          : *reinterpret_cast<const f32x4*>(a.pos ? a.pos + (size_t)(mc % a.tokens) * a.N + nc[j] : a.out_f32 + x_off(a, mc, nc[j], ld));
                }
#pragma unroll
                for (int u = 0; u < RB; ++u) {
                    if (i2 + u >= MR) continue;
                    const int m = m0 + wave_m * (MR * 16) + (i2 + u) * 16 + lr;
                    const int mcs = m < a.M ? m : a.M - 1;
#pragma unroll
                    for (int j = 0; j < 4; ++j) {
                        if constexpr (fold)
                            acc[i2 + u][j] = nv[j] ? xv[u][j] + (acc[i2 + u][j] * st[u].x + (bv[j] - uv[j] * st[u].y)) : f32x4{0.f, 0.f, 0.f, 0.f};
                        else if (a.res_scale)
                            acc[i2 + u][j] = nv[j] ? xv[u][j] * *reinterpret_cast<const f32x4*>(a.res_scale + nc[j]) + (acc[i2 + u][j] + bv[j])
                                                   : f32x4{0.f, 0.f, 0.f, 0.f};
                        else
                            acc[i2 + u][j] = nv[j] ? (a.pos ? acc[i2 + u][j] * a.qscale + bv[j] + xv[u][j] : xv[u][j] + (acc[i2 + u][j] + bv[j]))
                                                   : f32x4{0.f, 0.f, 0.f, 0.f};
                        if (nv[j] && m < a.M) *reinterpret_cast<f32x4*>(a.out_f32 + x_off(a, mcs, nc[j], ld)) = acc[i2 + u][j];
                    }
                }
                if (!copy) continue;
                if (a.stat_part) {
#pragma unroll
                    for (int u = 0; u < RB; ++u) {
                        const int i = i2 + u;
                        if (i >= MR) continue;
                        f32x4 t = acc[i][0], q = acc[i][0] * acc[i][0];
#pragma unroll
                        for (int j = 1; j < 4; ++j) {
                            t = t + acc[i][j];
                            q = q + acc[i][j] * acc[i][j];
                        }
                        float s1 = (t[0] + t[1]) + (t[2] + t[3]), s2 = (q[0] + q[1]) + (q[2] + q[3]);
                        s1 += __shfl_xor(s1, 16); s2 += __shfl_xor(s2, 16);
                        s1 += __shfl_xor(s1, 32); s2 += __shfl_xor(s2, 32);
                        if (lq == 0) red[(wave_m * (MR * 16) + i * 16 + lr) * 4 + wave_n] = make_float2(s1, s2);
                    }
                }
                staged_store_2blocks<F16>(image, lane, m0 + wave_m * (MR * 16) + i2 * 16, (MR - i2) < RB ? (MR - i2) : RB, a.M, a.out_bf16, ld, ncol0, a.N,
                                          [&](int u, int j) { return acc[i2 + u][j] * gv[j]; });
            }
            }
            if (copy && a.stat_part && finish_stats) {
                __builtin_amdgcn_fence(__ATOMIC_RELEASE, "workgroup");
                __builtin_amdgcn_s_barrier();
                __builtin_amdgcn_fence(__ATOMIC_ACQUIRE, "workgroup");
                const int t = wave_n * 64 + lane;
                if (t < MR * 16) {
                    const int r = wave_m * (MR * 16) + t;
                    const float2 p0 = red[r * 4], p1 = red[r * 4 + 1], p2 = red[r * 4 + 2], p3 = red[r * 4 + 3];
                    const int m = m0 + r;
                    if (m < a.M)
                        *reinterpret_cast<float2*>(a.stat_part + 2 * ((size_t)(n0 >> 8) * a.stat_stride + m)) =
                            make_float2((p0.x + p1.x) + (p2.x + p3.x), (p0.y + p1.y) + (p2.y + p3.y));
                }
            }
            return;
        }
        if constexpr (EPI == EPI_RESID || EPI == EPI_RESCALE || EPI == EPI_RESID_ROWSTAT || EPI == EPI_RESID_LS) {
            f32x4 rs[4];
            if constexpr (EPI == EPI_RESCALE) {
#pragma unroll
                for (int j = 0; j < 4; ++j) rs[j] = nv[j] ? *reinterpret_cast<const f32x4*>(a.res_scale + nc[j]) : f32x4{0.f, 0.f, 0.f, 0.f};
            }
            if constexpr (EPI == EPI_RESID_ROWSTAT) {
#pragma unroll
                for (int j = 0; j < 4; ++j) rs[j] = nv[j] ? *reinterpret_cast<const f32x4*>(a.col_u + nc[j]) : f32x4{0.f, 0.f, 0.f, 0.f};
            }
            constexpr int RB = 4;
            auto rmw = [&](auto interior_tag) {
                constexpr bool INTERIOR = decltype(interior_tag)::value;
#pragma unroll
                for (int i2 = 0; i2 < MR; i2 += RB) {
                    epi_turn(a, wave_m, i2 / RB);
                    f32x4 xv[RB][4];
#pragma unroll
                    for (int u = 0; u < RB; ++u) {
                        if (i2 + u >= MR) continue;
                        const int m = m0 + wave_m * (MR * 16) + (i2 + u) * 16 + lr;
                        const int mr = (INTERIOR || m < a.M) ? m : a.M - 1;
#pragma unroll
                        for (int j = 0; j < 4; ++j)
                            xv[u][j] = (INTERIOR || nv[j]) ? *reinterpret_cast<const f32x4*>(a.out_f32 + x_off(a, mr, nc[j], ld)) : f32x4{0.f, 0.f, 0.f, 0.f};
                    }
#pragma unroll
                    for (int u = 0; u < RB; ++u) {
                        if (i2 + u >= MR) continue;
                        const int m = m0 + wave_m * (MR * 16) + (i2 + u) * 16 + lr;
                        const int mc = (INTERIOR || m < a.M) ? m : a.M - 1;
                        float* row = (a.x_blocked && a.resid_rowmajor_out) ? a.resid_rowmajor_out + (size_t)mc * ld : nullptr;
                        float2 st = make_float2(1.f, 0.f);
                        if constexpr (EPI == EPI_RESID_ROWSTAT) st = st_lds ? st_lds[mc - m0] : row_stat(a, mc);
#pragma unroll
                        for (int j = 0; j < 4; ++j) {
                            f32x4 v;
                            if constexpr (EPI == EPI_RESCALE)
                                v = xv[u][j] * rs[j] + (acc[i2 + u][j] + bv[j]);
                            else if constexpr (EPI == EPI_RESID_ROWSTAT)
                                v = xv[u][j] + ((acc[i2 + u][j] * st.x - rs[j] * st.y) + bv[j]);
                            else if constexpr (EPI == EPI_RESID_LS)
                                v = xv[u][j] + ((INTERIOR || nv[j]) ? *reinterpret_cast<const f32x4*>(a.res_scale + nc[j]) : f32x4{0.f, 0.f, 0.f, 0.f}) *
                                                   (acc[i2 + u][j] + bv[j]);
                            else
                                v = xv[u][j] + (acc[i2 + u][j] + bv[j]);
                            if (INTERIOR || (nv[j] && m < a.M)) *reinterpret_cast<f32x4*>(row ? row + nc[j] : a.out_f32 + x_off(a, mc, nc[j], ld)) = v;
                            if constexpr (EPI == EPI_RESID_LS) {
                                if (a.out_bf16 && (INTERIOR || (nv[j] && m < a.M)))
                                    *reinterpret_cast<bf16x4*>(a.out_bf16 + (size_t)mc * ld + nc[j]) = pack4<F16>(v[0], v[1], v[2], v[3]);
                            }
                        }
                    }
                }
            };
            if (m0 + 2 * MR * 16 <= a.M && n0 + BN <= a.N) rmw(std::true_type{});
            else rmw(std::false_type{});
            return;
        }
        if constexpr (EPI == EPI_PATCH || EPI == EPI_BIAS) {
            if (m0 + 2 * MR * 16 <= a.M && n0 + BN <= a.N) {
#pragma unroll
                for (int i = 0; i < MR; ++i) {
                    const int m = m0 + wave_m * (MR * 16) + i * 16 + lr;
                    f32x4 pv[4];
                    if constexpr (EPI == EPI_PATCH) {
                        const int t = m % a.tokens;
#pragma unroll
                        for (int j = 0; j < 4; ++j) pv[j] = *reinterpret_cast<const f32x4*>(a.pos + (size_t)t * a.N + nc[j]);
                    }
#pragma unroll
                    for (int j = 0; j < 4; ++j) {
                        if constexpr (EPI == EPI_PATCH) *reinterpret_cast<f32x4*>(a.out_f32 + (size_t)m * ld + nc[j]) = acc[i][j] * a.qscale + bv[j] + pv[j];
                        else *reinterpret_cast<f32x4*>(a.out_f32 + x_off(a, m, nc[j], ld)) = acc[i][j] + bv[j];
                    }
                }
                return;
            }
        }
#pragma unroll
        for (int i = 0; i < MR; ++i) {
            const int m = m0 + wave_m * (MR * 16) + i * 16 + lr;
            if (m >= a.M) continue;
            if constexpr (EPI == EPI_PATCH) {
                const int t = m % a.tokens;
                f32x4 pv[4];
#pragma unroll
                for (int j = 0; j < 4; ++j)
                    pv[j] = nv[j] ? *reinterpret_cast<const f32x4*>(a.pos + (size_t)t * a.N + nc[j]) : f32x4{0.f, 0.f, 0.f, 0.f};
#pragma unroll
                for (int j = 0; j < 4; ++j)
                    if (nv[j]) *reinterpret_cast<f32x4*>(a.out_f32 + (size_t)m * ld + nc[j]) = acc[i][j] * a.qscale + bv[j] + pv[j];
            } else if constexpr (EPI == EPI_BIAS) {
#pragma unroll
                for (int j = 0; j < 4; ++j)
                    if (nv[j]) *reinterpret_cast<f32x4*>(a.out_f32 + x_off(a, m, nc[j], ld)) = acc[i][j] + bv[j];
            } else if constexpr (EPI == EPI_STAR) {
#pragma unroll
                for (int j = 0; j < 4; ++j) {
                    if (!nv[j]) continue;
                    const f32x4 v = star_relu4(acc[i][j] + bv[j], a.star_scale, a.star_bias, a.star_kind);
                    *reinterpret_cast<bf16x4*>(a.out_bf16 + (size_t)m * ld + nc[j]) = pack4<F16>(v[0], v[1], v[2], v[3]);
                }
            } else if constexpr (EPI == EPI_GELU) {
#pragma unroll
                for (int j = 0; j < 4; ++j) {
                    if (!nv[j]) continue;
                    const f32x4 v = acc[i][j] + bv[j];
                    const f32x4 gv = gelu_f4(v, a.gelu_tanh);
                    const bf16x4 o = pack4<F16>(gv[0], gv[1], gv[2], gv[3]);
                    *reinterpret_cast<bf16x4*>(a.out_bf16 + (size_t)m * ld + nc[j]) = o;
                }
            } else if constexpr (EPI == EPI_QK) {
                const int b = m / a.tokens, t = m - b * a.tokens;
#pragma unroll
                for (int j = 0; j < 4; ++j) {
                    if (!nv[j]) continue;
                    const int which = nc[j] >= 2 * a.dim ? 2 : (nc[j] >= a.dim ? 1 : 0);
                    const int nn = nc[j] - which * a.dim;
                    const int head = nn >> a.hd_log2, d = nn & ((1 << a.hd_log2) - 1);
                    const float sc = which ? 1.0f : a.qscale;
                    const f32x4 v = acc[i][j] + bv[j];
                    const bf16x4 o = pack4<F16>(v[0] * sc, v[1] * sc, v[2] * sc, v[3] * sc);
                    bf16_t* base = which == 2 ? a.out3_bf16 : (which ? a.out2_bf16 : a.out_bf16);
                    *reinterpret_cast<bf16x4*>(base + ((((size_t)(b * a.heads + head) * a.tokens_pad + t)) << a.hd_log2) + d) = o;
                }
            }
        }
    }
}

template <int EPI, int MR, bool F16>
__device__ __forceinline__ void gemm_epilogue_staged(const GemmArgs& a, f32x4 (&acc)[MR][4], int m0, int n0, int wave_m, int wave_n,
                                                     int lane, char* region, const f32x4* bias_pre = nullptr, const float2* st_lds = nullptr,
                                                     float2* red = nullptr) {
    f32x4 bias_v[4];
    if (bias_pre) {
#pragma unroll
        for (int j = 0; j < 4; ++j) bias_v[j] = bias_pre[j];
    } else {
        load_bias<EPI>(a, n0, wave_n, lane, bias_v);
    }
    static_assert(EPI == EPI_VT || EPI == EPI_GELU || EPI == EPI_STAR || EPI == EPI_QK || EPI == EPI_QK_ROPE || EPI == EPI_SWIGLU,
                  "staged epilogue: half-precision outputs only");
    constexpr bool IS_QK = EPI == EPI_QK || EPI == EPI_QK_ROPE;
    const bool fold = a.rowstat != nullptr || a.stat_in != nullptr;
    f32x4 cu[4];
    if (fold) load_cols<EPI>(a.col_u, a, n0, wave_n, lane, cu);
    else {
#pragma unroll
        for (int j = 0; j < 4; ++j) cu[j] = f32x4{0.f, 0.f, 0.f, 0.f};
    }
    const int lr = lane & 15, lq = lane >> 4;
    const int ncol0 = n0 + wave_n * 64;
    const int mrow0 = m0 + wave_m * (MR * 16);
    const int lc = lane & 7, lrow = lane >> 3;
    if constexpr (EPI == EPI_VT) {
        float bv[4];
#pragma unroll
        for (int j = 0; j < 4; ++j) bv[j] = bias_v[j][0];
#pragma unroll
        for (int pass = 0; pass < 2; ++pass) {
            if (pass) __builtin_amdgcn_wave_barrier();
#pragma unroll
            for (int ii = 0; ii < 4; ++ii) {
                const int i = pass * 4 + ii;
                if (i >= MR) continue;
                f32x4 sx{1.f, 1.f, 1.f, 1.f}, sy{0.f, 0.f, 0.f, 0.f};
                if (fold) {
                    const int mr = mrow0 + i * 16 + 4 * lq;
#pragma unroll
                    for (int e = 0; e < 4; ++e) {
                        const float2 st = st_lds ? st_lds[mr + e - m0] : row_stat(a, mr + e);
                        sx[e] = st.x;
                        sy[e] = st.y;
                    }
                }
#pragma unroll
                for (int j = 0; j < 4; ++j) {
                    const f32x4 c = acc[i][j] * sx + (bv[j] - sy * cu[j][0]);
                    const int d = j * 16 + lr;
                    const int pc = (ii * 2 + (lq >> 1)) ^ ((d >> 1) & 7);
                    *reinterpret_cast<bf16x4*>(region + d * 128 + pc * 16 + (lq & 1) * 8) = pack4<F16>(c[0], c[1], c[2], c[3]);
                }
            }
            __builtin_amdgcn_fence(__ATOMIC_RELEASE, "wavefront");
            __builtin_amdgcn_wave_barrier();
            const int m = mrow0 + pass * 64 + lc * 8;
            const int b = m / a.tokens, t = m - b * a.tokens;
            const bool mv = pass * 64 + lc * 8 < MR * 16 && m < a.M;
#pragma unroll
            for (int r8 = 0; r8 < 8; ++r8) {
                const int d = r8 * 8 + lrow;
                const int n = ncol0 + d;
                const uint4 v = *reinterpret_cast<const uint4*>(region + d * 128 + ((lc ^ ((d >> 1) & 7)) * 16));
                if (mv && n < a.N)
                    *reinterpret_cast<uint4*>(a.out_bf16 +
                                              ((((size_t)(b * a.heads + (n >> a.hd_log2))) << a.hd_log2) + (n & ((1 << a.hd_log2) - 1))) * a.tokens_pad + t) = v;
            }
            __builtin_amdgcn_fence(__ATOMIC_ACQUIRE, "wavefront");
        }
    } else {
        f32x4 bv[4];
#pragma unroll
        for (int j = 0; j < 4; ++j) bv[j] = bias_v[j];
        if constexpr (EPI == EPI_STAR) {
            if (a.out8) {
                staged_store_rows8<MR>(region, lane, mrow0, a.M, reinterpret_cast<uint8_t*>(a.out_bf16), a.ld_out ? a.ld_out : a.N, ncol0, a.N,
                                       [&](int i, int j) { return star_relu4(acc[i][j] + bv[j], a.star_scale, a.star_bias, a.star_kind); });
                return;
            }
        }
        if constexpr (EPI == EPI_SWIGLU) {
#pragma unroll
            for (int i = 0; i < MR; ++i) {
                float2 st = make_float2(1.f, 0.f);
                if (fold) st = st_lds ? st_lds[mrow0 - m0 + i * 16 + lr] : row_stat(a, mrow0 + i * 16 + lr);
#pragma unroll
                for (int jj = 0; jj < 2; ++jj)
                    acc[i][jj] = star_relu4(acc[i][jj] * st.x + (bv[jj] - cu[jj] * st.y), 0.f, 0.f, 1) *
                                 (acc[i][jj + 2] * st.x + (bv[jj + 2] - cu[jj + 2] * st.y));
                if (a.stat_part) {
                    const f32x4 t = acc[i][0] + acc[i][1], q = acc[i][0] * acc[i][0] + acc[i][1] * acc[i][1];
                    float s1 = (t[0] + t[1]) + (t[2] + t[3]), s2 = (q[0] + q[1]) + (q[2] + q[3]);
                    s1 += __shfl_xor(s1, 16); s2 += __shfl_xor(s2, 16);
                    s1 += __shfl_xor(s1, 32); s2 += __shfl_xor(s2, 32);
                    const int m = mrow0 + i * 16 + lr;
// ... 139 lines not shown
```

### anime-illust-image-searcher_amd/csrc/vit.hip

```cpp
#include <algorithm>
#include "../../include/hip_tagsearch_debug.h"
#include <cmath>
#include <cstdlib>
#include <cstdio>
#include <cstring>
#include <string>
#include <vector>

#include "vit_internal.h"
#include "model_host.h"
#include "row_ln.h"
#include "patch_rows.h"

using namespace hipts;

namespace {

struct Layer {
    DevBuf ln1_g, ln1_b, ln2_g, ln2_b;
    DevBuf qkv_w, qkv_b, proj_w, proj_b, fc1_w, fc1_b, fc2_w, fc2_b;
    DevBuf qkv_u, qkv_c, fc1_u, fc1_c;
};


// ... 703 lines not shown
}

int launch_layernorm(const float* x, const float* g, const float* b, bf16_t* out, int64_t rows, int D, float eps, bool f16,
                     hipStream_t s) {
    HIPTS_REQUIRE(D % 4 == 0 && D >= 4 && D <= 1024, "layernorm: D=%d must be a multiple of 4, at most 1024", D);
    const int blocks = (int)((rows + 3) / 4);
    const LnGammaOptBeta norm{g, b};
    HIPTS_LAUNCH_F16(f16, row_ln_kernel, blocks, 256, 0, s, FromF32{x}, norm, To16{out}, rows, D, eps);
    return HIPTS_OK;
}

int launch_layernorm8(const float* x, const float* g, const float* b, uint8_t* out, int64_t rows, int D, float eps, hipStream_t s) {
    HIPTS_REQUIRE(D % 4 == 0 && D >= 4 && D <= 1024, "layernorm: D=%d must be a multiple of 4, at most 1024", D);
    const int blocks = (int)((rows + 3) / 4);
    const LnGammaOptBeta norm{g, b};
    row_ln_kernel<false><<<blocks, 256, 0, s>>>(FromF32{x}, norm, ToE4m3{out}, rows, D, eps);
    HIPTS_LAUNCH_CHECK();
    return HIPTS_OK;
}
}

extern "C" {

int hipts_vit_set_sub_batches(hipts_vit_t* h, int n) {
    HIPTS_REQUIRE(h, "null handle");
    HIPTS_REQUIRE(n >= 0 && n <= hipts_vit::kMaxSub, "hipts_vit_set_sub_batches: n must be 0 .. %d", (int)hipts_vit::kMaxSub);
    h->want_sub = n;
    return HIPTS_OK;
}

int hipts_vit_set_deferred_join(hipts_vit_t* h, int on) {
    HIPTS_REQUIRE(h, "null handle");
    h->deferred_join = on != 0;
    return HIPTS_OK;
}

int hipts_vit_join(hipts_vit_t* h, void* stream) {
    HIPTS_REQUIRE(h, "null handle");
    HIPTS_TRY(use_device(h->device));
    for (int i = 0; i < h->last_ns; ++i) HIPTS_HIP(hipStreamWaitEvent((hipStream_t)stream, h->streams.ev_join[i], 0));
    return HIPTS_OK;
}

int hipts_vit_profile_enable(hipts_vit_t* h, int enable) {
    HIPTS_REQUIRE(h, "null handle");
    HIPTS_TRY(use_device(h->device));
    HIPTS_TRY(prof_resolve(h));
    for (int i = 0; i < PC_COUNT; ++i) {
        h->acc_ms[i] = h->acc_flops[i] = h->acc_bytes[i] = 0.0;
        h->acc_n[i] = 0;
    }
    h->prof_every = enable > 0 ? enable : 0;
    h->prof_calls = 0;
    h->prof = false;
    return HIPTS_OK;
}

int hipts_vit_profile_select(hipts_vit_t* h, uint32_t category_mask) {
    HIPTS_REQUIRE(h, "null handle");
    h->prof_mask = category_mask;
    return HIPTS_OK;
}

int hipts_vit_profile_read(hipts_vit_t* h, int category, double* total_ms, int64_t* launches, double* total_flops,
                           double* total_bytes) {
    HIPTS_REQUIRE(h && category >= 0 && category < PC_COUNT, "bad category");
    HIPTS_TRY(use_device(h->device));
    HIPTS_TRY(prof_resolve(h));
    if (total_ms) *total_ms = h->acc_ms[category];
    if (launches) *launches = h->acc_n[category];
    if (total_flops) *total_flops = h->acc_flops[category];
    if (total_bytes) *total_bytes = h->acc_bytes[category];
    return HIPTS_OK;
}

int hipts_vit_forward_u8(hipts_vit_t* h, const uint8_t* images, int images_memspace, int batch, float* logits_out,
                         float* probs_out, int out_memspace, void* stream) {
    return vit_forward_impl(h, images, images_memspace, true, batch, logits_out, probs_out, out_memspace, (hipStream_t)stream);
}

int hipts_vit_forward_f32(hipts_vit_t* h, const float* x, int x_memspace, int batch, float* logits_out, float* probs_out,
                          int out_memspace, void* stream) {
    return vit_forward_impl(h, x, x_memspace, false, batch, logits_out, probs_out, out_memspace, (hipStream_t)stream);
}

}

static float g_last_loop_ghz = 0.f;


extern "C" int hiptsdbg_gemm_clock(int M, int N, int K, int epi, int iters, float* ms_out, float* loop_ghz) {
    HIPTS_REQUIRE(ms_out && loop_ghz, "null argument");
    const char* had = getenv("HIPTS_GEMM_STAMPS");
    setenv("HIPTS_GEMM_STAMPS", "quiet", 1);
    g_last_loop_ghz = 0.f;
    const int st = hiptsdbg_gemm_time(M, N, K, epi, iters, ms_out);
    if (!had) unsetenv("HIPTS_GEMM_STAMPS");
    *loop_ghz = g_last_loop_ghz;
    return st;
}

extern "C" int hiptsdbg_gemm_time(int M, int N, int K, int epi, int iters, float* ms_out) {
    HIPTS_TRY(use_device(0));
    const int Np = round_up(N, 256);
    DevBuf A, W, bias, of32, obf, obf2, pos;
    HIPTS_TRY(A.alloc((size_t)M * K * 2));
    HIPTS_TRY(W.alloc((size_t)Np * K * 2));
    HIPTS_TRY(bias.alloc((size_t)Np * 4));
    HIPTS_TRY(of32.alloc((size_t)M * Np * 4));
    const size_t padded_rows = ((size_t)M / 784 + 1) * 832;
    const size_t obytes = (padded_rows > (size_t)M ? padded_rows : (size_t)M) * Np * 2 + (1 << 20);
    HIPTS_TRY(obf.alloc(obytes));
    HIPTS_TRY(obf2.alloc(obytes));
    HIPTS_TRY(pos.alloc((size_t)1024 * Np * 4));
    std::vector<uint16_t> ha((size_t)M * K), hw((size_t)Np * K);
    uint32_t st = 12345u;
    auto rnd = [&]() { st = st * 1664525u + 1013904223u; return ((st >> 8) & 0xffff) / 65536.0f * 2.0f - 1.0f; };
    const bool dbg_f16 = getenv("HIPTS_DBG_GEMM_F16") != nullptr;
    for (auto& v : ha) v = dbg_f16 ? f32_to_f16_rne(rnd()) : f32_to_bf16_rne(rnd());
    for (auto& v : hw) v = dbg_f16 ? f32_to_f16_rne(rnd() * 0.05f) : f32_to_bf16_rne(rnd() * 0.05f);
    if (getenv("HIPTS_DBG_GEMM_ZERO")) {
        for (auto& v : ha) v = 0;
        for (auto& v : hw) v = 0;
    }
    const bool op8 = getenv("HIPTS_GEMM_OP8") != nullptr;
    if (op8) {
        for (auto& v : ha) v &= 0xbfbf;
        for (auto& v : hw) v &= 0xbfbf;
    }
    HIPTS_TRY(upload(A.p, ha.data(), ha.size() * 2));
    HIPTS_TRY(upload(W.p, hw.data(), hw.size() * 2));
    HIPTS_HIP(hipMemset(bias.p, 0, bias.bytes));
    HIPTS_HIP(hipMemset(of32.p, 0, of32.bytes));
    HIPTS_HIP(hipMemset(pos.p, 0, pos.bytes));
    GemmArgs g{};
    g.A = A.as<bf16_t>(); g.W = W.as<bf16_t>(); g.M = M; g.N = N; g.K = K; g.bias = bias.as<float>();
    g.out_f32 = of32.as<float>(); g.out_bf16 = obf.as<bf16_t>(); g.out2_bf16 = obf2.as<bf16_t>(); g.pos = pos.as<float>();
    g.tokens = 784; g.tokens_pad = 832; g.heads = N / 128 > 0 ? N / 128 : 1; g.dim = N / 2; g.qscale = 0.125f;
    if (epi == EPI_VT) { g.heads = N / 64; g.dim = N; }
    DevBuf statp;
    if (epi == EPI_RESID_XG) {
        HIPTS_TRY(statp.alloc((size_t)(Np / 256) * M * 8));
        g.pos = nullptr; g.ln_gamma = bias.as<float>(); g.stat_part = statp.as<float>(); g.stat_stride = M;
    }
    if (op8) { g.op8 = 1; g.f16 = 1; g.w_exp = 3; g.out8 = (epi == EPI_STAR && getenv("HIPTS_GEMM_OUT8")) ? 1 : 0; }
    if (dbg_f16) g.f16 = 1;
    if (getenv("HIPTS_DBG_X_BLOCKED")) g.x_blocked = 1;
    if (getenv("HIPTS_DBG_GEMM_SHARED")) g.shared_chip = 1;
    if (epi == EPI_QK && N % 3 == 0) { g.dim = N / 3; g.heads = g.dim / 64; g.out3_bf16 = obf2.as<bf16_t>(); }
    DevBuf stamps;
    if (getenv("HIPTS_GEMM_STAMPS")) {
        HIPTS_TRY(stamps.alloc(4096 * 8 * 8));
        HIPTS_HIP(hipMemset(stamps.p, 0, 4096 * 8 * 8));
        g.stamps = stamps.as<unsigned long long>();
        g.trace = getenv("HIPTS_GEMM_TRACE") ? 1 : 0;
    }
    hipEvent_t e0, e1;
    HIPTS_HIP(hipEventCreate(&e0));
    HIPTS_HIP(hipEventCreate(&e1));
    DevBuf skws;
    if (getenv("HIPTS_DBG_GEMM_SK")) {
        HIPTS_TRY(skws.alloc(GEMM_SK_WS_BYTES));
        HIPTS_HIP(hipMemset(skws.p, 0, skws.bytes));
        g.sk_ws = skws.p; g.sk_ws_bytes = GEMM_SK_WS_BYTES; g.shared_chip = 1;
    }
    for (int i = 0; i < 3; ++i) HIPTS_TRY(launch_gemm((GemmEpilogue)epi, g, nullptr));
    HIPTS_HIP(hipEventRecord(e0, nullptr));
    for (int i = 0; i < iters; ++i) HIPTS_TRY(launch_gemm((GemmEpilogue)epi, g, nullptr));
    HIPTS_HIP(hipEventRecord(e1, nullptr));
    HIPTS_HIP(hipEventSynchronize(e1));
    float ms = 0.f;
    HIPTS_HIP(hipEventElapsedTime(&ms, e0, e1));
    *ms_out = ms / iters;
    if (g.stamps) {
        unsigned long long h[8 * 64];
        HIPTS_HIP(hipMemcpy(h, g.stamps, sizeof(h), hipMemcpyDeviceToHost));
        unsigned long long base = ~0ull;
        for (int w = 0; w < 8; ++w) if (h[w * 64] && h[w * 64] < base) base = h[w * 64];
        if (gemm_q4_launch_count() > 0 && getenv("HIPTS_GEMM_Q4")) {
            fprintf(stderr, "4-wave loop, workgroup 8: per tile start -> loop | loop (phase 0 | wait + barrier | phase 1) | epilogue, cycles\n");
            for (int w = 0; w < 4; ++w)
                for (int t = 0; t < 8; ++t) {
                    const unsigned long long* o = h + w * 64 + t * 8;
                    if (!o[0]) continue;
                    fprintf(stderr, "wave %d tile %d: top +%6lld  start %5lld  loop %7lld (p0 %7lld | wait %6lld | p1 %7lld)  epilogue %6lld  clock %.2f GHz\n", w, t,
                            (long long)(o[0] - base), (long long)(o[1] - o[0]), (long long)(o[2] - o[1]), (long long)o[4], (long long)o[5], (long long)o[6],
                            (long long)(o[3] - o[2]), o[7] ? (o[2] - o[1]) / (o[7] * 10.0) : 0.0);
                }
        } else
        if (getenv("HIPTS_GEMM_TRACE")) {
            std::vector<unsigned long long> tr(4096 * 8);
            HIPTS_HIP(hipMemcpy(tr.data(), g.stamps, tr.size() * 8, hipMemcpyDeviceToHost));
            FILE* f = fopen(getenv("HIPTS_GEMM_TRACE"), "w");
            if (f) {
                for (int b = 0; b < 4096; ++b)
                    if (tr[b * 8 + 2])
                        fprintf(f, "%d %llu %llu %llu %llu %llu\n", b, tr[b * 8], tr[b * 8 + 1], tr[b * 8 + 2], tr[b * 8 + 3], tr[b * 8 + 4]);
                fclose(f);
            }
        } else
        if (getenv("HIPTS_GEMM") && strcmp(getenv("HIPTS_GEMM"), "dw") == 0) {
            for (int w = 0; w < 4; ++w)
                fprintf(stderr, "dw wave %d: loop %lld cycles, waitcnt %lld, barrier %lld, wall %lld x 10 ns -> %.2f GHz\n", w, (long long)h[w * 64],
                        (long long)h[w * 64 + 1], (long long)h[w * 64 + 2], (long long)h[w * 64 + 3], h[w * 64] / (h[w * 64 + 3] * 10.0));
        }
        const bool quiet = strcmp(getenv("HIPTS_GEMM_STAMPS"), "quiet") == 0 || getenv("HIPTS_GEMM_TRACE") ||
                           (getenv("HIPTS_GEMM") && strcmp(getenv("HIPTS_GEMM"), "dw") == 0);
        if (h[2] && h[7] > h[6]) g_last_loop_ghz = (float)((h[3] - h[2]) / ((h[7] - h[6]) * 10.0));
        if (!quiet) fprintf(stderr, "stamps of workgroup 8 (cycles since first): per tile [top, K-tile 0 landed, loop start, loop end, next prologue issued, epilogue issued]\n");
        for (int w = 0; w < 8 && !quiet; w += 4) {
            for (int t = 0; t < 8; ++t) {
                if (!h[w * 64 + t * 8]) continue;
                fprintf(stderr, "wave %d tile %d:", w, t);
                for (int i = 0; i < 6; ++i) fprintf(stderr, " %7lld", (long long)(h[w * 64 + t * 8 + i] - base));
                fprintf(stderr, "  loop clock %.2f GHz", (h[w * 64 + t * 8 + 3] - h[w * 64 + t * 8 + 2]) / ((h[w * 64 + t * 8 + 7] - h[w * 64 + t * 8 + 6]) * 10.0));
                fprintf(stderr, "\n");
            }
        }
    }
    (void)hipEventDestroy(e0);
    (void)hipEventDestroy(e1);
    return HIPTS_OK;
}

extern "C" int hiptsdbg_gemm_q4_compare(int M, int N, int K, int epi, int f16, int iters, long long* mismatch_out, float* ms_out) {
    HIPTS_TRY(use_device(0));
    HIPTS_REQUIRE(mismatch_out && ms_out && (epi == EPI_GELU || epi == EPI_QK || epi == EPI_RESID_XG), "hiptsdbg_gemm_q4_compare: epilogue %d", epi);
    HIPTS_REQUIRE(M % 256 == 0 && N % 256 == 0 && K % 128 == 0 && M % 784 == 0, "hiptsdbg_gemm_q4_compare: whole tiles, even K-tile count, whole images");
    DevBuf A, W, bias, gamma, x0, of32, obf[3], statp;
    HIPTS_TRY(A.alloc((size_t)M * K * 2));
    HIPTS_TRY(W.alloc((size_t)N * K * 2));
    HIPTS_TRY(bias.alloc((size_t)N * 4));
    HIPTS_TRY(gamma.alloc((size_t)N * 4));
    HIPTS_TRY(x0.alloc((size_t)M * N * 4));
    HIPTS_TRY(of32.alloc((size_t)M * N * 4));
    const size_t obytes = ((size_t)M / 784) * 832 * N * 2 + (1 << 20);
    for (auto& b : obf) HIPTS_TRY(b.alloc(obytes));
    HIPTS_TRY(statp.alloc((size_t)(N / 256) * M * 8));
    {
        std::vector<uint16_t> ha((size_t)M * K), hw((size_t)N * K);
        std::vector<float> hb((size_t)N), hg((size_t)N), hx((size_t)M * N);
        uint32_t st = 2468u + (uint32_t)(M + 3 * N + 7 * K);
        auto rnd = [&]() { st = st * 1664525u + 1013904223u; return ((st >> 8) & 0xffff) / 65536.0f * 2.0f - 1.0f; };
        for (auto& v : ha) v = f16 ? f32_to_f16_rne(rnd()) : f32_to_bf16_rne(rnd());
        for (auto& v : hw) v = f16 ? f32_to_f16_rne(rnd() * 0.05f) : f32_to_bf16_rne(rnd() * 0.05f);
        for (auto& v : hb) v = rnd() * 0.3f;
        for (auto& v : hg) v = 1.0f + rnd() * 0.2f;
        for (auto& v : hx) v = rnd() * 3.0f;
        HIPTS_TRY(upload(A.p, ha.data(), ha.size() * 2));
        HIPTS_TRY(upload(W.p, hw.data(), hw.size() * 2));
        HIPTS_TRY(upload(bias.p, hb.data(), hb.size() * 4));
        HIPTS_TRY(upload(gamma.p, hg.data(), hg.size() * 4));
        HIPTS_TRY(upload(x0.p, hx.data(), hx.size() * 4));
    }
    GemmArgs g{};
    g.A = A.as<bf16_t>(); g.W = W.as<bf16_t>(); g.M = M; g.N = N; g.K = K; g.bias = bias.as<float>(); g.f16 = f16 ? 1 : 0;
    g.out_f32 = of32.as<float>(); g.out_bf16 = obf[0].as<bf16_t>(); g.out2_bf16 = obf[1].as<bf16_t>();
    g.tokens = 784; g.tokens_pad = 832; g.qscale = 0.125f;
    if (epi == EPI_QK) {
        if (N % 3 == 0) { g.dim = N / 3; g.out3_bf16 = obf[2].as<bf16_t>(); } else g.dim = N / 2;
        g.heads = g.dim / 64;
        HIPTS_REQUIRE(g.dim % 64 == 0, "hiptsdbg_gemm_q4_compare: q | k | v widths must be multiples of 64");
    }
    if (epi == EPI_RESID_XG) { g.ln_gamma = gamma.as<float>(); g.stat_part = statp.as<float>(); g.stat_stride = M; }
    g.shared_chip = 1;
    const long long q4_before = gemm_q4_launch_count();
    std::vector<std::vector<char>> keep[2];
    hipEvent_t e0, e1;
    HIPTS_HIP(hipEventCreate(&e0));
    HIPTS_HIP(hipEventCreate(&e1));
    const unsigned mask_before = 0;
    (void)mask_before;
    for (int pass = 0; pass < 2; ++pass) {
        set_gemm_q4_mask(pass ? (1u << epi) : 0u);
        HIPTS_HIP(hipMemcpy(of32.p, x0.p, of32.bytes, hipMemcpyDeviceToDevice));
        for (auto& b : obf) HIPTS_HIP(hipMemset(b.p, 0, b.bytes));
        HIPTS_HIP(hipMemset(statp.p, 0, statp.bytes));
        HIPTS_TRY(launch_gemm((GemmEpilogue)epi, g, nullptr));
        HIPTS_HIP(hipDeviceSynchronize());
        DevBuf* outs[5] = {&of32, &obf[0], &obf[1], &obf[2], &statp};
        for (DevBuf* b : outs) {
            keep[pass].emplace_back(b->bytes);
            HIPTS_HIP(hipMemcpy(keep[pass].back().data(), b->p, b->bytes, hipMemcpyDeviceToHost));
        }
        HIPTS_HIP(hipEventRecord(e0, nullptr));
        for (int i = 0; i < iters; ++i) HIPTS_TRY(launch_gemm((GemmEpilogue)epi, g, nullptr));
        HIPTS_HIP(hipEventRecord(e1, nullptr));
        HIPTS_HIP(hipEventSynchronize(e1));
        float ms = 0.f;
        HIPTS_HIP(hipEventElapsedTime(&ms, e0, e1));
        ms_out[pass] = iters > 0 ? ms / iters : 0.f;
    }
    set_gemm_q4_mask(getenv("HIPTS_GEMM_Q4") ? (unsigned)strtoul(getenv("HIPTS_GEMM_Q4"), nullptr, 0) : GEMM_Q4_DEFAULT_MASK);
    (void)hipEventDestroy(e0);
    (void)hipEventDestroy(e1);
    HIPTS_REQUIRE(gemm_q4_launch_count() == q4_before + 1 + iters, "hiptsdbg_gemm_q4_compare: the launcher did not take the 4-wave loop for this shape");
    long long bad = 0;
    for (size_t b = 0; b < keep[0].size(); ++b)
        for (size_t i = 0; i < keep[0][b].size(); ++i) bad += keep[0][b][i] != keep[1][b][i];
    *mismatch_out = bad;
    return HIPTS_OK;
}

extern "C" int hiptsdbg_gemm_run(int M, int N, int K, const uint16_t* a_bf16, const uint16_t* w_bf16, float* out_host) {
    HIPTS_TRY(use_device(0));
    HIPTS_REQUIRE(M >= 1 && N >= 16 && N % 16 == 0 && K >= 64 && K % 64 == 0, "hiptsdbg_gemm_run: unsupported shape");
    const int Np = round_up(N, 256);
    DevBuf A, W, bias, out;
    HIPTS_TRY(A.alloc((size_t)M * K * 2));
    HIPTS_TRY(W.alloc((size_t)Np * K * 2));
    HIPTS_TRY(bias.alloc((size_t)Np * 4));
    HIPTS_TRY(out.alloc((size_t)M * N * 4));
    HIPTS_HIP(hipMemset(W.p, 0, W.bytes));
    HIPTS_HIP(hipMemset(bias.p, 0, bias.bytes));
    HIPTS_HIP(hipMemset(out.p, 0, out.bytes));
    HIPTS_TRY(upload(A.p, a_bf16, (size_t)M * K * 2));
    HIPTS_TRY(upload(W.p, w_bf16, (size_t)N * K * 2));
    GemmArgs g{};
    g.A = A.as<bf16_t>(); g.W = W.as<bf16_t>(); g.M = M; g.N = N; g.K = K; g.bias = bias.as<float>(); g.out_f32 = out.as<float>();
    g.f16 = getenv("HIPTS_DBG_GEMM_F16") ? 1 : 0;
    DevBuf skws;
    if (getenv("HIPTS_DBG_GEMM_SK")) {
        HIPTS_TRY(skws.alloc(GEMM_SK_WS_BYTES));
        HIPTS_HIP(hipMemset(skws.p, 0, skws.bytes));
        g.sk_ws = skws.p; g.sk_ws_bytes = GEMM_SK_WS_BYTES; g.shared_chip = 1;
    }
    HIPTS_TRY(launch_gemm(EPI_RESID, g, nullptr));
    if (skws.p) HIPTS_TRY(launch_gemm(EPI_RESID, g, nullptr));
    if (skws.p) {
        std::vector<unsigned> tk(1024);
        HIPTS_HIP(hipMemcpy(tk.data(), skws.p, 4096, hipMemcpyDeviceToHost));
        for (unsigned v : tk) HIPTS_REQUIRE(v == 0, "hiptsdbg_gemm_run: a split-K ticket was left at %u", v);
    }
    HIPTS_HIP(hipMemcpy(out_host, out.p, (size_t)M * N * 4, hipMemcpyDeviceToHost));
    return HIPTS_OK;
}

extern "C" int hiptsdbg_gemm8_run(int M, int N, int K, const float* a_f32, const float* w_f32, int kind, void* out_host, int* w_exp) {
    HIPTS_TRY(use_device(0));
    HIPTS_REQUIRE(M >= 1 && N >= 16 && N % 16 == 0 && K >= 128 && K % 128 == 0 && w_exp, "hiptsdbg_gemm8_run: unsupported shape");
    const int Np = round_up(N, 256);
    DevBuf A, W, bias, out;
    HIPTS_TRY(A.alloc((size_t)M * K));
    std::vector<uint8_t> ha((size_t)M * K);
    for (size_t i = 0; i < ha.size(); ++i) ha[i] = f32_to_e4m3_rne(a_f32[i]);
    HIPTS_TRY(upload(A.p, ha.data(), ha.size()));
    HIPTS_TRY(upload_matrix8(W, w_f32, N, K, Np, w_exp));
    HIPTS_TRY(bias.alloc((size_t)Np * 4));
    HIPTS_TRY(out.alloc((size_t)M * N * 4));
    HIPTS_HIP(hipMemset(bias.p, 0, bias.bytes));
    HIPTS_HIP(hipMemset(out.p, 0, out.bytes));
    GemmArgs g{};
    g.A = A.as<bf16_t>(); g.W = W.as<bf16_t>(); g.M = M; g.N = N; g.K = K; g.bias = bias.as<float>();
    g.f16 = 1; g.op8 = 1; g.w_exp = *w_exp;
    if (kind == 0) {
        g.out_f32 = out.as<float>();
        HIPTS_TRY(launch_gemm(EPI_RESID, g, nullptr));
        HIPTS_HIP(hipMemcpy(out_host, out.p, (size_t)M * N * 4, hipMemcpyDeviceToHost));
    } else {
        g.out_bf16 = out.as<bf16_t>(); g.out8 = 1; g.star_kind = 2;
        HIPTS_TRY(launch_gemm(EPI_STAR, g, nullptr));
        HIPTS_HIP(hipMemcpy(out_host, out.p, (size_t)M * N, hipMemcpyDeviceToHost));
    }
    return HIPTS_OK;
}

extern "C" int hiptsdbg_attention_run(const uint16_t* q, const uint16_t* k, const uint16_t* vT, uint16_t* out_host, int batch, int heads, int tokens,
                                      int tokens_pad, int head_dim, int f16) {
    HIPTS_REQUIRE(q && k && vT && out_host && batch >= 1 && heads >= 1 && tokens >= 1, "hiptsdbg_attention_run: bad arguments");
    HIPTS_TRY(use_device(0));
    const size_t nqk = (size_t)batch * heads * tokens_pad * head_dim, nout = (size_t)batch * tokens * heads * head_dim;
    DevBuf dq, dk, dv, dout;
    HIPTS_TRY(dq.alloc(nqk * 2));
    HIPTS_TRY(dk.alloc(nqk * 2));
    HIPTS_TRY(dv.alloc(nqk * 2));
    HIPTS_TRY(dout.alloc(nout * 2));
    HIPTS_TRY(upload(dq.p, q, nqk * 2));
    HIPTS_TRY(upload(dk.p, k, nqk * 2));
    HIPTS_TRY(upload(dv.p, vT, nqk * 2));
    HIPTS_HIP(hipMemset(dout.p, 0, nout * 2));
    HIPTS_TRY(launch_attention(dq.as<bf16_t>(), dk.as<bf16_t>(), dv.as<bf16_t>(), dout.as<bf16_t>(), batch, heads, tokens, tokens_pad, f16 != 0, nullptr,
                               head_dim, 0));
    HIPTS_HIP(hipDeviceSynchronize());
    HIPTS_HIP(hipMemcpy(out_host, dout.p, nout * 2, hipMemcpyDeviceToHost));
    return HIPTS_OK;
}

extern "C" int hiptsdbg_attention_time(const uint16_t* q, const uint16_t* k, const uint16_t* vT, int batch, int heads, int tokens, int tokens_pad,
                                       int head_dim, int f16, int iters, double* avg_us) {
    HIPTS_REQUIRE(q && k && vT && avg_us && batch >= 1 && heads >= 1 && tokens >= 1 && iters >= 1, "hiptsdbg_attention_time: bad arguments");
    HIPTS_TRY(use_device(0));
    const size_t nqk = (size_t)batch * heads * tokens_pad * head_dim, nout = (size_t)batch * tokens * heads * head_dim;
    DevBuf dq, dk, dv, dout;
    HIPTS_TRY(dq.alloc(nqk * 2));
    HIPTS_TRY(dk.alloc(nqk * 2));
    HIPTS_TRY(dv.alloc(nqk * 2));
    HIPTS_TRY(dout.alloc(nout * 2));
    HIPTS_TRY(upload(dq.p, q, nqk * 2));
    HIPTS_TRY(upload(dk.p, k, nqk * 2));
    HIPTS_TRY(upload(dv.p, vT, nqk * 2));
    hipEvent_t e0, e1;
    HIPTS_HIP(hipEventCreate(&e0));
    HIPTS_HIP(hipEventCreate(&e1));
    int rc = HIPTS_OK;
    for (int i = 0; i < 3 && rc == HIPTS_OK; ++i)
        rc = launch_attention(dq.as<bf16_t>(), dk.as<bf16_t>(), dv.as<bf16_t>(), dout.as<bf16_t>(), batch, heads, tokens, tokens_pad, f16 != 0, nullptr, head_dim, 0);
    HIPTS_HIP(hipEventRecord(e0, nullptr));
    for (int i = 0; i < iters && rc == HIPTS_OK; ++i)
        rc = launch_attention(dq.as<bf16_t>(), dk.as<bf16_t>(), dv.as<bf16_t>(), dout.as<bf16_t>(), batch, heads, tokens, tokens_pad, f16 != 0, nullptr, head_dim, 0);
    HIPTS_HIP(hipEventRecord(e1, nullptr));
    HIPTS_HIP(hipEventSynchronize(e1));
    float ms = 0.f;
    HIPTS_HIP(hipEventElapsedTime(&ms, e0, e1));
    (void)hipEventDestroy(e0);
    (void)hipEventDestroy(e1);
    *avg_us = 1e3 * ms / iters;
    return rc;
}

extern "C" int hiptsdbg_attention2(const uint16_t* q, const uint16_t* k, const uint16_t* v, uint16_t* out_host, int batch, int heads, int tokens,
                                   int tokens_pad, int f16, int variant, int iters, double* avg_us) {
    HIPTS_REQUIRE(q && k && v && batch >= 1 && heads >= 1 && tokens >= 1 && (iters > 0 ? avg_us != nullptr : out_host != nullptr), "hiptsdbg_attention2: bad arguments");
    HIPTS_TRY(use_device(0));
    const size_t nqk = (size_t)batch * heads * tokens_pad * 64, nout = (size_t)batch * tokens * heads * 64;
    DevBuf dq, dk, dv, dout;
    HIPTS_TRY(dq.alloc(nqk * 2));
    HIPTS_TRY(dk.alloc(nqk * 2));
    HIPTS_TRY(dv.alloc(nqk * 2));
    HIPTS_TRY(dout.alloc(nout * 2));
    HIPTS_TRY(upload(dq.p, q, nqk * 2));
    HIPTS_TRY(upload(dk.p, k, nqk * 2));
    HIPTS_TRY(upload(dv.p, v, nqk * 2));
    HIPTS_HIP(hipMemset(dout.p, 0, nout * 2));
    auto run = [&]() { return launch_attention2(dq.as<bf16_t>(), dk.as<bf16_t>(), dv.as<bf16_t>(), dout.as<bf16_t>(), batch, heads, tokens, tokens_pad, f16 != 0, nullptr, 0, variant); };
    if (iters <= 0) {
        HIPTS_TRY(run());
        HIPTS_HIP(hipDeviceSynchronize());
        HIPTS_HIP(hipMemcpy(out_host, dout.p, nout * 2, hipMemcpyDeviceToHost));
        return HIPTS_OK;
    }
    hipEvent_t e0, e1;
    HIPTS_HIP(hipEventCreate(&e0));
    HIPTS_HIP(hipEventCreate(&e1));
    int rc = HIPTS_OK;
    for (int i = 0; i < 3 && rc == HIPTS_OK; ++i) rc = run();
    HIPTS_HIP(hipEventRecord(e0, nullptr));
    for (int i = 0; i < iters && rc == HIPTS_OK; ++i) rc = run();
    HIPTS_HIP(hipEventRecord(e1, nullptr));
    HIPTS_HIP(hipEventSynchronize(e1));
    float ms = 0.f;
    HIPTS_HIP(hipEventElapsedTime(&ms, e0, e1));
    (void)hipEventDestroy(e0);
    (void)hipEventDestroy(e1);
    *avg_us = 1e3 * ms / iters;
    return rc;
}

extern "C" int hiptsdbg_attention2_stamps(unsigned long long* host, int n) { return attention2_read_stamps(host, n); }

extern "C" int hiptsdbg_vit_dump(hipts_vit_t* h, const char* name, void* out_host, size_t max_bytes, size_t* bytes) {
    HIPTS_REQUIRE(h && name && out_host && bytes, "null argument");
    HIPTS_TRY(use_device(h->device));
    const std::string n(name);
    const DevBuf* b = n == "a0" ? &h->a0 : n == "x" ? &h->x : n == "xn" ? &h->xn : n == "q" ? &h->q : n == "k" ? &h->k
                      : n == "v" ? &h->v : n == "att" ? &h->att : n == "hmid" ? &h->hmid : n == "pool_part" ? &h->pool_part
                      : n == "pooled2" ? &h->pooled2 : nullptr;
    HIPTS_REQUIRE(b, "unknown buffer %s", name);
    *bytes = b->bytes < max_bytes ? b->bytes : max_bytes;
    HIPTS_HIP(hipDeviceSynchronize());
    HIPTS_HIP(hipMemcpy(out_host, b->p, *bytes, hipMemcpyDeviceToHost));
    return HIPTS_OK;
}
```

### anime-illust-image-searcher_amd/csrc/vit_internal.h

```cpp
#pragma once
#include <cmath>
#include <cstring>
#include <vector>

#include "common.h"

namespace hipts {

typedef __bf16 bf16_t;
typedef __bf16 bf16x8 __attribute__((ext_vector_type(8)));
typedef __bf16 bf16x4 __attribute__((ext_vector_type(4)));
typedef _Float16 f16x8 __attribute__((ext_vector_type(8)));
typedef _Float16 f16x4 __attribute__((ext_vector_type(4)));
typedef float f32x4 __attribute__((ext_vector_type(4)));
typedef float f32x16 __attribute__((ext_vector_type(16)));
typedef int i32x8 __attribute__((ext_vector_type(8)));

template <bool F16>
__device__ __forceinline__ bf16x4 pack4(float a, float b, float c, float d) {
    if constexpr (F16) {
        f16x4 h;
        h[0] = (_Float16)a; h[1] = (_Float16)b; h[2] = (_Float16)c; h[3] = (_Float16)d;
        return __builtin_bit_cast(bf16x4, h);
    } else {
        bf16x4 o;
        o[0] = (bf16_t)a; o[1] = (bf16_t)b; o[2] = (bf16_t)c; o[3] = (bf16_t)d;
        return o;
    }
}
template <bool F16>
__device__ __forceinline__ bf16_t to_op(float a) {
    if constexpr (F16) return __builtin_bit_cast(bf16_t, (_Float16)a);
    else return (bf16_t)a;
}
template <bool F16>
__device__ __forceinline__ float from_op(bf16_t a) {
    if constexpr (F16) return (float)__builtin_bit_cast(_Float16, a);
    else return (float)a;
}
template <bool F16>
__device__ __forceinline__ f32x4 mfma_16x16x32(bf16x8 a, bf16x8 b, f32x4 c) {
    if constexpr (F16) return __builtin_amdgcn_mfma_f32_16x16x32_f16(__builtin_bit_cast(f16x8, a), __builtin_bit_cast(f16x8, b), c, 0, 0, 0);
    else return __builtin_amdgcn_mfma_f32_16x16x32_bf16(a, b, c, 0, 0, 0);
}
template <bool F16>
__device__ __forceinline__ f32x16 mfma_32x32x16(bf16x8 a, bf16x8 b, f32x16 c) {
    if constexpr (F16) return __builtin_amdgcn_mfma_f32_32x32x16_f16(__builtin_bit_cast(f16x8, a), __builtin_bit_cast(f16x8, b), c, 0, 0, 0);
    else return __builtin_amdgcn_mfma_f32_32x32x16_bf16(a, b, c, 0, 0, 0);
}

__device__ __forceinline__ uint32_t pack4_e4m3(float a, float b, float c, float d) {
    a = __builtin_amdgcn_fmed3f(a, -448.0f, 448.0f);
    b = __builtin_amdgcn_fmed3f(b, -448.0f, 448.0f);
    c = __builtin_amdgcn_fmed3f(c, -448.0f, 448.0f);
    d = __builtin_amdgcn_fmed3f(d, -448.0f, 448.0f);
    int p = __builtin_amdgcn_cvt_pk_fp8_f32(a, b, 0, false);
    p = __builtin_amdgcn_cvt_pk_fp8_f32(c, d, p, true);
    return (uint32_t)p;
}
__device__ __forceinline__ f32x4 mfma_16x16x128_e4m3(i32x8 a, i32x8 b, f32x4 c, int scale_a, int scale_b) {
    return __builtin_amdgcn_mfma_scale_f32_16x16x128_f8f6f4(a, b, c, 0, 0, 0, scale_a, 0, scale_b);
}

inline uint8_t f32_to_e4m3_rne(float f) {
    uint32_t u;
    memcpy(&u, &f, 4);
    const uint8_t sign = (uint8_t)((u >> 24) & 0x80u);
    u &= 0x7fffffffu;
    if (u > 0x7f800000u) return (uint8_t)(sign | 0x7f);
    float a;
    memcpy(&a, &u, 4);
    if (a >= 448.0f) return (uint8_t)(sign | 0x7e);
    if (a < 0.0009765625f) return sign;
    int e;
    (void)frexpf(a, &e);
    int ex = e - 1;
    if (ex < -6) ex = -6;
    const float q = ldexpf(1.0f, ex - 3);
    const float n = nearbyintf(a / q);
    float v = n * q;
    if (v >= 448.0f) return (uint8_t)(sign | 0x7e);
    if (v < 0.015625f) return (uint8_t)(sign | (uint8_t)n);
    int e2;
    const float m2 = frexpf(v, &e2);
    const int bexp = e2 - 1 + 7;
    const int mant = (int)((m2 * 2.0f - 1.0f) * 8.0f);
    return (uint8_t)(sign | (bexp << 3) | mant);
}
inline float e4m3_bits_to_f32(uint8_t v) {
    const int s = v >> 7, e = (v >> 3) & 15, m = v & 7;
    float f;
    if (e == 15 && m == 7) {
        const uint32_t qnan = 0x7fc00000u;
        memcpy(&f, &qnan, 4);
    } else if (e == 0) f = ldexpf((float)m, -9);
    else f = ldexpf(1.0f + (float)m / 8.0f, e - 7);
    return s ? -f : f;
}
inline uint16_t f32_to_bf16_rne(float f) {
    uint32_t u;
    memcpy(&u, &f, 4);
    if ((u & 0x7fffffffu) > 0x7f800000u) return (uint16_t)((u >> 16) | 0x40);
    u += 0x7fffu + ((u >> 16) & 1u);
    return (uint16_t)(u >> 16);
}

inline uint16_t f32_to_f16_rne(float f) {
    uint32_t x;
    memcpy(&x, &f, 4);
    const uint32_t sign = (x >> 16) & 0x8000u;
    x &= 0x7fffffffu;
    if (x >= 0x7f800000u) return (uint16_t)(sign | 0x7c00u | (x > 0x7f800000u ? 0x200u : 0));
    if (x >= 0x477ff000u) return (uint16_t)(sign | 0x7c00u);
    if (x < 0x38800000u) {
        if (x < 0x33000000u) return (uint16_t)sign;
        const int shift = 126 - (int)(x >> 23);
        uint32_t mant = (x & 0x7fffffu) | 0x800000u;
        const uint32_t round = (1u << (shift - 1)) - 1 + ((mant >> shift) & 1u);
        mant += round;
        return (uint16_t)(sign | (mant >> shift));
    }
    const uint32_t round = 0xfffu + ((x >> 13) & 1u);
    x += round;
    return (uint16_t)(sign | ((x - 0x38000000u) >> 13));
}
inline float f16_bits_to_f32(uint16_t h) {
    const uint32_t sign = (uint32_t)(h & 0x8000u) << 16;
    uint32_t e = (h >> 10) & 0x1f, m = h & 0x3ffu, out;
    if (e == 0) {
        if (m == 0) out = sign;
        else {
            int sh = 0;
            while (!(m & 0x400u)) { m <<= 1; ++sh; }
            out = sign | ((uint32_t)(113 - sh) << 23) | ((m & 0x3ffu) << 13);
        }
    } else if (e == 31) out = sign | 0x7f800000u | (m << 13);
    else out = sign | ((e + 112) << 23) | (m << 13);
    float f;
    memcpy(&f, &out, 4);
    return f;
}

inline int round_up(int x, int m) { return (x + m - 1) / m * m; }

inline int upload_matrix16(DevBuf& buf, const float* data, int rows, int cols, int rows_pad, bool f16) {
    std::vector<uint16_t> h((size_t)rows_pad * cols, 0);
    if (f16) for (size_t i = 0; i < (size_t)rows * cols; ++i) h[i] = f32_to_f16_rne(data[i]);
    else for (size_t i = 0; i < (size_t)rows * cols; ++i) h[i] = f32_to_bf16_rne(data[i]);
    HIPTS_TRY(buf.alloc(h.size() * 2));
    return upload(buf.p, h.data(), h.size() * 2);
}

inline int upload_matrix8(DevBuf& buf, const float* data, int rows, int cols, int rows_pad, int* w_exp) {
    float mx = 0.f;
    for (size_t i = 0; i < (size_t)rows * cols; ++i) mx = fmaxf(mx, fabsf(data[i]));
    int e = 0;
    if (mx > 0.f && std::isfinite(mx)) {
        e = (int)floorf(log2f(448.0f / mx));
        if (ldexpf(mx, e) > 448.0f) --e;
        e = e > 100 ? 100 : (e < -100 ? -100 : e);
    }
    std::vector<uint8_t> h((size_t)rows_pad * cols, 0);
    for (size_t i = 0; i < (size_t)rows * cols; ++i) h[i] = f32_to_e4m3_rne(ldexpf(data[i], e));
    *w_exp = e;
    HIPTS_TRY(buf.alloc(h.size()));
    return upload(buf.p, h.data(), h.size());
}

enum GemmEpilogue {
    EPI_PATCH = 0,
    EPI_QK = 1,
    EPI_VT = 2,
    EPI_RESID = 3,
    EPI_GELU = 4,
    EPI_HEAD = 5,
    EPI_STAR = 6,
    EPI_RESCALE = 7,
    EPI_BIAS = 8,
    EPI_QK_ROPE = 10,
    EPI_SWIGLU = 11,
    EPI_RESID_ROWSTAT = 12,
    EPI_RESID_XG = 13,
    EPI_RESID_XGI = 14,
    EPI_RESID_LS = 15,
    EPI_RESID_LN = 9
};

struct GemmArgs {
    const bf16_t* A;
    const bf16_t* W;
    int M, N, K;
    const float* bias;
    float* out_f32 = nullptr;
    float* out2_f32 = nullptr;
    bf16_t* out_bf16 = nullptr;
    bf16_t* out2_bf16 = nullptr;
    bf16_t* out3_bf16 = nullptr;
    const float* pos = nullptr;
    int tokens = 0;
    int tokens_pad = 0;
    int heads = 0, dim = 0;
    int hd_log2 = 6;
    const float* res_scale = nullptr;
    const float* ln_gamma = nullptr;
    const float* ln_beta = nullptr;
    float ln_eps = 1e-6f;
    float star_scale = 1.0f, star_bias = 0.0f;
    int star_kind = 0;
    float qscale = 1.0f;
    float* stat_part = nullptr;
    int stat_stride = 0;
    const float* stat_in = nullptr;
    int stat_in_blocks = 0;
    int stat_in_stride = 0;
    int ln_dim = 0;
    const float* rowstat = nullptr;
    const float* col_u = nullptr;
    const float* rope = nullptr;
    int rope_tokens = 0;
    int gelu_tanh = 1;
    int ld_out = 0;
    int f16 = 0;
    int op8 = 0;
    int w_exp = 0;
    int out8 = 0;
    void* sk_ws = nullptr;
    size_t sk_ws_bytes = 0;
    int sk_first = 0, sk_slices = 1;
    int raster_gn = 0;
    int raster_gm = 0;
    int x_blocked = 0;
    float* resid_rowmajor_out = nullptr;
    int epi_prefetch = 0;
    int epi_prio = 0;
    int shared_chip = 0;
    int trace = 0;
    unsigned long long* stamps = nullptr;
};

int launch_gemm(GemmEpilogue epi, const GemmArgs& a, hipStream_t s);
int launch_gemm_q4(GemmEpilogue epi, const GemmArgs& a, hipStream_t s, bool* handled);
constexpr unsigned GEMM_Q4_DEFAULT_MASK = 0u;
void set_gemm_q4_mask(unsigned mask);
long long gemm_q4_launch_count();
constexpr size_t GEMM_SK_WS_BYTES = 4096 + 256 * (size_t)(256 * 256 * 4);

int launch_attention(const bf16_t* q, const bf16_t* k, const bf16_t* vT, bf16_t* out, int batch, int heads, int tokens,
                     int tokens_pad, bool f16, hipStream_t s, int head_dim = 64, int out_tokens_stride = 0);

int launch_attention2(const bf16_t* q, const bf16_t* k, const bf16_t* v, bf16_t* out, int batch, int heads, int tokens, int tokens_pad, bool f16,
                      hipStream_t s, int out_tokens_stride = 0, int variant = 0, int split_lo = 0, float lo_scale = 1.0f);
inline float split_lo_scale(bool f16) {
    static const float env = getenv("HIPTS_SPLIT_LO_SCALE") ? (float)atof(getenv("HIPTS_SPLIT_LO_SCALE")) : 0.0f;
    if (env > 0.0f) return env;
    return f16 ? 64.0f : 1.0f;
}

int attention2_read_stamps(unsigned long long* host, int n);

int launch_swin_attention(const float* qkv, const float* logit_scale, const float* cpb, bf16_t* out, int batch, int side, int window,
                          int shift, int heads, bool f16, hipStream_t s);

int launch_layernorm(const float* x, const float* g, const float* b, bf16_t* out, int64_t rows, int D, float eps, bool f16,
                     hipStream_t s);
int launch_rowstat(const float* part, float* rowstat, int M, int stride, int blocks, int D, float eps, hipStream_t s);
int launch_fold_ln(const bf16_t* W, bool f16, const float* gamma, const float* beta, const float* bias, float* u, float* c, int N, int K,
                   hipStream_t s);
std::vector<uint16_t> mlp_weight_image(const float* w1, const float* w2, int C);
bool mlp_fused_supports(int C);
int launch_mlp_fused(const bf16_t* xn, const void* wimg, float* x, const float* res_scale, const float* gamma, bf16_t* xn_out, int M, int C,
                     float star_s, float star_b, float eps, hipStream_t s, int waves = 0,
                     int xblk = 0);
int launch_layernorm8(const float* x, const float* g, const float* b, uint8_t* out, int64_t rows, int D, float eps, hipStream_t s);

}
```

### include/hip_tagsearch_debug.h

```cpp
#ifndef HIP_TAGSEARCH_DEBUG_H
#define HIP_TAGSEARCH_DEBUG_H

#include <stddef.h>
#include <stdint.h>

#include "hip_tagsearch.h"

#ifdef __cplusplus
extern "C" {
#endif

int hiptsdbg_gemm_time(int M, int N, int K, int epi, int iters, float* ms_out);
int hiptsdbg_gemm_clock(int M, int N, int K, int epi, int iters, float* ms_out, float* loop_ghz);
int hiptsdbg_gemm_q4_compare(int M, int N, int K, int epi, int f16, int iters, long long* mismatch_out, float* ms_out);
int hiptsdbg_gelu(const float* x_host, int n, int tanh_form, float* y_host);
int hiptsdbg_dwconv7(const uint16_t* in_f16, const float* w, uint16_t* out_f16, int batch, int H, int C, int mode, int iters, float* ms_out);
int hiptsdbg_dwconv7_stamps(unsigned long long* host, int n);
int hiptsdbg_convnext_stream(hipts_convnext_t* h, const float* x_host, int batch, int stage, float* out_host);
int hiptsdbg_swinv2_stream(hipts_swinv2_t* h, const float* x_host, int batch, int stage, float* out_host);
int hiptsdbg_swinv2_window_attention(const float* q, const float* k, const float* v, const float* logit_scale, const float* cpb, int batch,
                                     int heads, int side, int window, int shift, int operand_f16, float* out);
int hiptsdbg_mlp_fused(const uint16_t* xn, const float* w1, const float* w2, float* x, const float* res_scale, const float* gamma, uint16_t* xn_out,
                       int M, int C, float star_s, float star_b, float eps, int iters, float* ms_out, int waves);
int hiptsdbg_mlp_stamps(unsigned long long* host, int n);
int hiptsdbg_mlp_weight_image(const float* w1, const float* w2, int C, uint16_t* out, long long out_halves);
int hiptsdbg_dw_toeplitz(const float* w, int channels, uint32_t* out);
int hiptsdbg_gemm_run(int M, int N, int K, const uint16_t* a_bf16, const uint16_t* w_bf16, float* out_host);
int hiptsdbg_gemm8_run(int M, int N, int K, const float* a_f32, const float* w_f32, int kind, void* out_host, int* w_exp);
int hiptsdbg_vit_dump(hipts_vit_t* h, const char* name, void* out_host, size_t max_bytes, size_t* bytes);

int hiptsdbg_attention_run(const uint16_t* q, const uint16_t* k, const uint16_t* vT, uint16_t* out_host, int batch, int heads, int tokens,
                           int tokens_pad, int head_dim, int f16);
int hiptsdbg_attention_time(const uint16_t* q, const uint16_t* k, const uint16_t* vT, int batch, int heads, int tokens, int tokens_pad,
                            int head_dim, int f16, int iters, double* avg_us);

int hiptsdbg_attention2(const uint16_t* q, const uint16_t* k, const uint16_t* v, uint16_t* out_host, int batch, int heads, int tokens, int tokens_pad,
                        int f16, int variant, int iters, double* avg_us);

int hiptsdbg_attention2_stamps(unsigned long long* host, int n);

int hiptsdbg_search1_last(hipts_bm25_t* h, uint32_t* candidates, uint32_t* took_candidate_path);
int hiptsdbg_topk_stamps(unsigned long long* host16);

#ifdef __cplusplus
}
#endif
#endif
```

Measured before the change: 5430 images/sec.

## Split persistent GEMM tail-wave tiles into half-height pieces for residual epilogues

When a persistent residual GEMM's tile count leaves a partial last wave, the remaining 256-row tiles are split into two 128-row pieces so more CUs share the tail work. The kernel gains a TP template path that runs items at height 4 or 8 via a generic run_item lambda, with staging, MFMA loops and epilogues parameterised on that height. This targets the idle-CU cost of the final wave, at the price of extra code size, register pressure and a more complex scheduling path. It is enabled by default on exclusive chips through an env-controlled switch.

```diff
diff --git a/anime-illust-image-searcher_amd/csrc/gemm.hip b/anime-illust-image-searcher_amd/csrc/gemm.hip
--- a/anime-illust-image-searcher_amd/csrc/gemm.hip
+++ b/anime-illust-image-searcher_amd/csrc/gemm.hip
@@ -94,11 +94,12 @@
     }
 }
 
-template <int EPI, int MR = 8, bool F16 = false, bool OP8 = false, bool SK = false, bool INT = false>
+template <int EPI, int MR = 8, bool F16 = false, bool OP8 = false, bool SK = false, bool INT = false, bool TP = false>
 __global__ __launch_bounds__(512) __attribute__((amdgpu_num_vgpr(HIPTS_INT_DEPTH == 3 ? 256 : 240))) void gemm_pp_kernel(const GemmArgs a, int tiles_m, int tiles_n) {
     static_assert(!INT || (EPI == EPI_RESID_XG && MR == 8 && !OP8 && !SK), "INT: the residual epilogue's interior form");
     static_assert(!OP8 || (F16 && MR == 8), "e4m3 operands: half 16-bit outputs, full tiles");
     static_assert(!SK || (!OP8 && MR == 8), "split-K: 16-bit operands, full tiles");
+    static_assert(!TP || (!OP8 && !SK && MR == 8 && HIPTS_STAGE_AHEAD && !HIPTS_STAGE_ORDER_OLD), "half-height tail: 16-bit operands, full tiles, the staging-ahead order");
     constexpr int TBM = 2 * MR * 16;
     extern __shared__ __attribute__((aligned(16))) char smem[];
     __shared__ float2 st_table[256];
@@ -133,7 +134,14 @@
     const int K = OP8 ? a.K / 2 : a.K, nt_all = K / BK;
     const int w_rows = tiles_n * BN;
     const int S = SK ? a.sk_slices : 1;
-    const int n_items = SK ? a.sk_first + (nwg - a.sk_first) * S : nwg;
+    const int tp_rem = TP ? nwg - a.tp_first : 0;
+    const int n_items = TP ? a.tp_first + 16 * (tp_rem >> 3) + ((tp_rem & 7) ? 8 + (tp_rem & 7) : 0) : SK ? a.sk_first + (nwg - a.sk_first) * S : nwg;
+    auto piece_of = [&](int item, int& tid_, int& half_) {
+        const int j = item - a.tp_first, tl = (j >> 4) * 8 + (j & 7);
+        tid_ = a.tp_first + tl;
+        half_ = (j >> 3) & 1;
+        return tl < tp_rem;
+    };
     auto decode = [&](int item, int& tid_, int& slice_, int& kt0_, int& ntl_) {
         if (!SK || item < a.sk_first) {
             tid_ = item; slice_ = -1; kt0_ = 0; ntl_ = nt_all;
@@ -159,11 +167,33 @@
     } while (0)
     int tile = blockIdx.x, m0, n0;
     int tix, slice, kt0, nt;
-    decode(tile, tix, slice, kt0, nt);
-    tile_origin(tix, m0, n0);
+    int half = -1;
+    auto locate = [&](int& it, int& tix_, int& slice_, int& kt0_, int& nt_, int& m0_, int& n0_, int& half_) {
+        half_ = -1;
+        if constexpr (TP) {
+            for (; it < n_items; it += gridDim.x) {
+                if (it < a.tp_first) break;
+                if (!piece_of(it, tix_, half_)) continue;
+                tile_origin(tix_, m0_, n0_);
+                m0_ += half_ * (TBM / 2);
+                if (m0_ < a.M) {
+                    slice_ = -1; kt0_ = 0; nt_ = nt_all;
+                    return true;
+                }
+            }
+            half_ = -1;
+            if (it >= n_items) return false;
+        } else if (it >= n_items) {
+            return false;
+        }
+        decode(it, tix_, slice_, kt0_, nt_);
+        tile_origin(tix_, m0_, n0_);
+        return true;
+    };
+    if (!locate(tile, tix, slice, kt0, nt, m0, n0, half)) return;
     int par = 0;
 
-    if (wave * 4 < 4 * MR) stage_tile(a.A, a.M, K, m0, kt0, smem, wave, lane);
+    if (wave * 4 < 4 * (half >= 0 ? MR / 2 : MR)) stage_tile(a.A, a.M, K, m0, kt0, smem, wave, lane);
     stage_tile(a.W, w_rows, K, n0, kt0, smem + TILE_BYTES, wave, lane);
     if constexpr (INT) {
         for (int i = tid; i < (a.N >> 2); i += 512) {
@@ -174,10 +204,12 @@
         asm volatile("s_waitcnt lgkmcnt(0)" ::: "memory");
     }
 
-    for (;;) {
-        f32x4 acc[MR][4];
-#pragma unroll
-        for (int i = 0; i < MR; ++i)
+    auto run_item = [&](auto height) __attribute__((always_inline)) -> bool {
+        constexpr int H = decltype(height)::value;
+        constexpr int HBM = 2 * H * 16;
+        f32x4 acc[H][4];
+#pragma unroll
+        for (int i = 0; i < H; ++i)
 #pragma unroll
             for (int j = 0; j < 4; ++j) acc[i][j] = f32x4{0.f, 0.f, 0.f, 0.f};
 
@@ -197,20 +229,25 @@
                 const int e = 2 * wave + u;
                 slot(0 + u, true, e);
                 slot(2 + u, true, 16 + e);
-                slot(4 + u, false, e < 8 ? e : 2 * MR + (e - 8));
-            }
-            if constexpr (MR == 8) {
+                slot(4 + u, false, e < 8 ? e : 2 * H + (e - 8));
+            }
+            if constexpr (H == 4) {
+                for (int k = 6; k < 8; ++k) {
+                    src[k] = src[4];
+                    dst[k] = dst[4];
+                }
+            } else if constexpr (H == 8) {
                 for (int u = 0; u < 2; ++u) {
                     const int e = 2 * wave + u;
-                    slot(6 + u, false, e < 8 ? 8 + e : 2 * MR + 8 + (e - 8));
-                }
-            } else if constexpr (MR == 6) {
-                slot(6, false, wave < 4 ? 8 + wave : 2 * MR + 8 + (wave - 4));
+                    slot(6 + u, false, e < 8 ? 8 + e : 2 * H + 8 + (e - 8));
+                }
+            } else if constexpr (H == 6) {
+                slot(6, false, wave < 4 ? 8 + wave : 2 * H + 8 + (wave - 4));
                 src[7] = src[6];
                 dst[7] = dst[6];
             } else {
-                static_assert(MR == 7, "tile heights: 256, 224 or 192 rows");
-                auto hi = [](int f) { return f < 6 ? 8 + f : 2 * MR + 8 + (f - 6); };
+                static_assert(H == 7, "tile heights: 256, 224 or 192 rows");
+                auto hi = [](int f) { return f < 6 ? 8 + f : 2 * H + 8 + (f - 6); };
                 if (wave < 4) {
                     slot(6, false, hi(2 * wave));
                     slot(7, false, hi(2 * wave + 1));
@@ -221,7 +258,7 @@
                 }
             }
         }
-        const int n_hi = (MR == 8 || (MR == 7 && wave < 4)) ? 2 : 1;
+        const int n_hi = H == 4 ? 0 : (H == 8 || (H == 7 && wave < 4)) ? 2 : 1;
         PPSTAMP(0);
         asm volatile("s_waitcnt vmcnt(0)" ::: "memory");
         PPSTAMP(1);
@@ -255,7 +292,7 @@
                     }
                     if (kk == 0) {
 #pragma unroll
-                        for (int i = 0; i < 4; ++i) af8[i] = read_frag8(cur, wave_m * MR + mh * 4 + i, lane);
+                        for (int i = 0; i < 4; ++i) af8[i] = read_frag8(cur, wave_m * H + mh * 4 + i, lane);
                     }
                 } else {
                 if (p < 2) {
@@ -264,7 +301,7 @@
                 }
 #pragma unroll
                 for (int i = 0; i < 4; ++i)
-                    if (mh * 4 + i < MR) af[i] = read_frag(cur, wave_m * MR + mh * 4 + i, kk, lane);
+                    if (mh * 4 + i < H) af[i] = read_frag(cur, wave_m * H + mh * 4 + i, kk, lane);
                 }
                 if (more) {
                     auto issue = [&](int k) {
@@ -284,7 +321,7 @@
                         if (p == 0) {
                             issue(2); issue(3);
                         } else if (p == 1) {
-                            issue(6);
+                            if (n_hi >= 1) issue(6);
                             if (n_hi == 2) issue(7);
                             wait_vmcnt(6 + n_hi);
                         } else if (p == 3) {
@@ -316,7 +353,7 @@
                 } else if (p == 1) {
                     asm volatile("s_waitcnt vmcnt(0)" ::: "memory");
                 }
-                if constexpr (INT) {
+                if constexpr (INT && H == 8) {
                     if (!more && p == 2 && a.epi_prefetch) {
                         const int ldx = a.ld_out ? a.ld_out : a.N;
                         const char* xb = reinterpret_cast<const char*>(a.out_f32 + (size_t)(m0 + wave_m * 128) * ldx + n0 + wave_n * 64);
@@ -354,7 +391,7 @@
 #else
                     const int i = ij >> 2, j = ij & 3;
 #endif
-                    if (mh * 4 + i >= MR) continue;
+                    if (mh * 4 + i >= H) continue;
                     if constexpr (EPI == EPI_VT)
                         acc[mh * 4 + i][j] = mfma_16x16x32<F16>(af[i], wf[kk][j], acc[mh * 4 + i][j]);
                     else
@@ -383,23 +420,21 @@
         const bool fold_st = FOLDABLE && a.stat_in != nullptr;
         const bool fold_many = fold_st && a.stat_in_blocks > 4;
         float2 st_pv[4];
-        if (fold_st && !fold_many && tid < TBM) row_stat_request(a, m0 + tid, st_pv);
-        const int next = tile + gridDim.x;
-        const bool has_next = next < n_items;
-        int m0n = 0, n0n = 0, tixn = 0, slicen = -1, kt0n = 0, ntn = nt_all;
+        if (fold_st && !fold_many && tid < HBM) row_stat_request(a, m0 + tid, st_pv);
+        int next = tile + gridDim.x;
+        int m0n = 0, n0n = 0, tixn = 0, slicen = -1, kt0n = 0, ntn = nt_all, halfn = -1;
+        const bool has_next = locate(next, tixn, slicen, kt0n, ntn, m0n, n0n, halfn);
         const int par_next = (par + nt) & 1;
         if (has_next) {
-            decode(next, tixn, slicen, kt0n, ntn);
-            tile_origin(tixn, m0n, n0n);
             char* st = smem + par_next * STAGE_BYTES;
-            if (wave * 4 < 4 * MR) stage_tile(a.A, a.M, K, m0n, kt0n, st, wave, lane);
+            if (wave * 4 < 4 * (TP ? (halfn >= 0 ? 4 : 8) : H)) stage_tile(a.A, a.M, K, m0n, kt0n, st, wave, lane);
             stage_tile(a.W, w_rows, K, n0n, kt0n, st + TILE_BYTES, wave, lane);
         }
         PPSTAMP(4);
         bool run_epilogue = true;
         if constexpr (SK) {
             if (slice >= 0) {
-                constexpr size_t SLAB = (size_t)TBM * BN * 4;
+                constexpr size_t SLAB = (size_t)HBM * BN * 4;
                 const int tl = tix - a.sk_first;
                 unsigned* tickets = reinterpret_cast<unsigned*>(a.sk_ws);
                 char* slabs = reinterpret_cast<char*>(a.sk_ws) + 4096 + (size_t)tl * S * SLAB;
@@ -407,10 +442,10 @@
                     const auto rs = __builtin_amdgcn_make_buffer_rsrc(slabs + (size_t)slice * SLAB, 0, (int)SLAB, 0x00020000);
                     typedef unsigned int u32x4 __attribute__((ext_vector_type(4)));
 #pragma unroll
-                    for (int i = 0; i < MR; ++i)
+                    for (int i = 0; i < H; ++i)
 #pragma unroll
                         for (int j = 0; j < 4; ++j)
-                            __builtin_amdgcn_raw_buffer_store_b128(__builtin_bit_cast(u32x4, acc[i][j]), rs, (((wave * MR + i) * 4 + j) * 64 + lane) * 16, 0, 16);
+                            __builtin_amdgcn_raw_buffer_store_b128(__builtin_bit_cast(u32x4, acc[i][j]), rs, (((wave * H + i) * 4 + j) * 64 + lane) * 16, 0, 16);
                 }
                 asm volatile("s_waitcnt vmcnt(0)" ::: "memory");
                 __builtin_amdgcn_s_barrier();
@@ -429,9 +464,9 @@
                     }
                     asm volatile("s_waitcnt vmcnt(0)" ::: "memory");
                     __builtin_amdgcn_s_barrier();
-                    const f32x4* sl = reinterpret_cast<const f32x4*>(slabs) + (size_t)(wave * MR * 4) * 64 + lane;
-#pragma unroll
-                    for (int i = 0; i < MR; ++i) {
+                    const f32x4* sl = reinterpret_cast<const f32x4*>(slabs) + (size_t)(wave * H * 4) * 64 + lane;
+#pragma unroll
+                    for (int i = 0; i < H; ++i) {
 #pragma unroll
                         for (int j = 0; j < 4; ++j) acc[i][j] = sl[(size_t)(i * 4 + j) * 64];
                         for (int sx = 1; sx < S; ++sx) {
@@ -449,8 +484,8 @@
         if (run_epilogue) {
         if (fold_st) {
             if (fold_many) {
-                if (tid < TBM) st_table[tid] = row_stat(a, m0 + tid);
-            } else if (tid < TBM) st_table[tid] = row_stat_finish(a, st_pv);
+                if (tid < HBM) st_table[tid] = row_stat(a, m0 + tid);
+            } else if (tid < HBM) st_table[tid] = row_stat_finish(a, st_pv);
             __builtin_amdgcn_fence(__ATOMIC_RELEASE, "workgroup");
             __builtin_amdgcn_s_barrier();
             __builtin_amdgcn_fence(__ATOMIC_ACQUIRE, "workgroup");
@@ -462,7 +497,7 @@
                                                                      : ((a.ld_out ? a.ld_out : a.N) % 8 == 0);
             if (ok) {
                 float2* red = (EPI == EPI_SWIGLU && a.stat_part) ? sw_red : nullptr;
-                gemm_epilogue_staged<EPI, MR, F16>(a, acc, m0, n0, wave_m, wave_n, lane,
+                gemm_epilogue_staged<EPI, H, F16>(a, acc, m0, n0, wave_m, wave_n, lane,
                                                    smem + ((par + nt + 1) & 1) * STAGE_BYTES + wave * 8192, bias_pre, fold_st ? st_table : nullptr, red);
                 staged = true;
                 if constexpr (EPI == EPI_SWIGLU) {
@@ -470,7 +505,7 @@
                         __builtin_amdgcn_fence(__ATOMIC_RELEASE, "workgroup");
                         __builtin_amdgcn_s_barrier();
                         __builtin_amdgcn_fence(__ATOMIC_ACQUIRE, "workgroup");
-                        if (tid < TBM) {
+                        if (tid < HBM) {
                             const float2 p0 = red[tid * 4], p1 = red[tid * 4 + 1], p2 = red[tid * 4 + 2], p3 = red[tid * 4 + 3];
                             const int m = m0 + tid;
                             if (m < a.M)
@@ -482,14 +517,14 @@
             }
         }
         if (!staged)
-            gemm_epilogue<EPI, MR, F16, INT>(a, acc, m0, n0, wave_m, wave_n, lane, bias_pre, smem + ((par + nt + 1) & 1) * STAGE_BYTES,
+            gemm_epilogue<EPI, H, F16, INT>(a, acc, m0, n0, wave_m, wave_n, lane, bias_pre, smem + ((par + nt + 1) & 1) * STAGE_BYTES,
                                              fold_st ? st_table : nullptr, INT ? colvec : nullptr);
         }
         if (a.epi_prio) __builtin_amdgcn_s_setprio(0);
         if constexpr (INT) asm volatile("" ::"v"(xpf));
         PPSTAMP(5);
         ++stamp_tile;
-        if (!has_next) break;
+        if (!has_next) return false;
         tile = next;
         tix = tixn;
         slice = slicen;
@@ -497,7 +532,15 @@
         nt = ntn;
         m0 = m0n;
         n0 = n0n;
+        half = halfn;
         par = par_next;
+        return true;
+    };
+    for (;;) {
+        bool more;
+        if constexpr (TP) more = half >= 0 ? run_item(std::integral_constant<int, 4>{}) : run_item(std::integral_constant<int, 8>{});
+        else more = run_item(std::integral_constant<int, MR>{});
+        if (!more) break;
     }
 }
 
@@ -903,6 +946,21 @@
     return (unsigned)v;
 }
 
+constexpr bool TAIL_PIECES_BUILT = HIPTS_STAGE_AHEAD && !HIPTS_STAGE_ORDER_OLD;
+constexpr int TAIL_PIECES_SHARED_DEFAULT = 0;
+constexpr int TAIL_PIECES_EXCLUSIVE_DEFAULT = 1;
+std::atomic<int> g_tail_pieces{-2};
+bool gemm_tail_pieces(bool shared_chip) {
+    int v = g_tail_pieces.load(std::memory_order_relaxed);
+    if (v == -2) {
+        v = getenv("HIPTS_GEMM_TAIL_PIECES") ? (atoi(getenv("HIPTS_GEMM_TAIL_PIECES")) != 0 ? 1 : 0) : -1;
+        g_tail_pieces.store(v, std::memory_order_relaxed);
+    }
+    return v >= 0 ? v != 0 : (shared_chip ? TAIL_PIECES_SHARED_DEFAULT : TAIL_PIECES_EXCLUSIVE_DEFAULT) != 0;
+}
+std::atomic<int> g_slots_override{0};
+thread_local int g_last_items = 0;
+
 int gemm_variant() {
     static int v = -1;
     if (v < 0) {
@@ -915,7 +973,9 @@
 template <int EPI>
 int launch_t(const GemmArgs& a, hipStream_t s) {
     int dev = 0;
-    const int cus_dev = current_device_cus(&dev);
+    int cus_dev = current_device_cus(&dev);
+    const int slots_forced = g_slots_override.load(std::memory_order_relaxed);
+    if (slots_forced > 0) cus_dev = slots_forced;
     static PerDevice attr;
     {
       std::lock_guard<std::mutex> lk(attr.mu);
@@ -1013,7 +1073,7 @@
             const int tiles_mr = tiles_of(mr);
             static const bool persist = !(getenv("HIPTS_GEMM_PERSIST") && strcmp(getenv("HIPTS_GEMM_PERSIST"), "0") == 0);
             const int ntile = tiles_mr * tiles_n;
-            const int slots = cus >= 8 ? cus / 8 * 8 : cus;
+            const int slots = slots_forced > 0 ? slots_forced : cus >= 8 ? cus / 8 * 8 : cus;
             const int grid = (persist && ntile > slots) ? slots : ntile;
             static const int raster = getenv("HIPTS_GEMM_RASTER") ? atoi(getenv("HIPTS_GEMM_RASTER")) : 8;
             static const int raster_gn = getenv("HIPTS_GEMM_RASTER_GN") ? atoi(getenv("HIPTS_GEMM_RASTER_GN")) : 6;
@@ -1064,8 +1124,65 @@
                     }
                 }
             }
+            g_last_items = ntile;
+            bool pieces = false;
+            if constexpr (TAIL_PIECES_BUILT && (EPI == EPI_RESID || EPI == EPI_RESID_XG || EPI == EPI_RESID_XGI || EPI == EPI_RESID_ROWSTAT)) {
+                const int rem = ntile % slots;
+                if (mr == 8 && persist && rem > 0 && 2 * rem <= slots && gemm_tail_pieces(a.shared_chip != 0)) {
+                    pieces = true;
+                    ar.tp_first = ntile - rem;
+                    int n_piece = 2 * rem;
+                    if (a.M <= (tiles_m - 1) * BM + BM / 2) {
+                        for (int id = ar.tp_first; id < ntile; ++id) {
+                            const int q = ntile >> 3, r = ntile & 7, xcd = id & 7, loc = id >> 3;
+                            const int bid = (xcd < r ? xcd * (q + 1) : r * (q + 1) + (xcd - r) * q) + loc;
+                            int panel = bid / tiles_n;
+                            if (ar.raster_gn > 0) {
+                                const int per = tiles_m * ar.raster_gn, grp = bid / per, left = tiles_n - grp * ar.raster_gn;
+                                panel = (bid - grp * per) / (left < ar.raster_gn ? left : ar.raster_gn);
+                            } else if (ar.raster_gm > 0) {
+                                const int per = ar.raster_gm * tiles_n, grp = bid / per, left = tiles_m - grp * ar.raster_gm;
+                                panel = grp * ar.raster_gm + (bid - grp * per) % (left < ar.raster_gm ? left : ar.raster_gm);
+                            }
+                            n_piece -= panel == tiles_m - 1;
+                        }
+                    }
+                    const int span = 16 * (rem >> 3) + ((rem & 7) ? 8 + (rem & 7) : 0);
+                    const int grid_tp = ar.tp_first + span > slots ? slots : ar.tp_first + span;
+                    g_last_items = ar.tp_first + n_piece;
+                    bool interior = false;
+                    if constexpr (EPI == EPI_RESID_XG)
+                        interior = a.M % 256 == 0 && a.N % 256 == 0 && a.N <= 1024 && !a.pos && !a.res_scale && a.out_bf16 && a.stat_part && !resid_general && !a.resid_general;
+                    static PerDevice attr_tp;
+                    {
+                        std::lock_guard<std::mutex> lk(attr_tp.mu);
+                        if (!attr_tp.done(dev)) {
+                            HIPTS_HIP(hipFuncSetAttribute((const void*)gemm_pp_kernel<EPI, 8, false, false, false, false, true>, hipFuncAttributeMaxDynamicSharedMemorySize, LDS_BYTES));
+                            HIPTS_HIP(hipFuncSetAttribute((const void*)gemm_pp_kernel<EPI, 8, true, false, false, false, true>, hipFuncAttributeMaxDynamicSharedMemorySize, LDS_BYTES));
+                            if constexpr (EPI == EPI_RESID_XG) {
+                                HIPTS_HIP(hipFuncSetAttribute((const void*)gemm_pp_kernel<EPI, 8, false, false, false, true, true>, hipFuncAttributeMaxDynamicSharedMemorySize, LDS_BYTES));
+                                HIPTS_HIP(hipFuncSetAttribute((const void*)gemm_pp_kernel<EPI, 8, true, false, false, true, true>, hipFuncAttributeMaxDynamicSharedMemorySize, LDS_BYTES));
+                            }
+                            attr_tp.mark(dev);
+                        }
+                    }
+                    if constexpr (EPI == EPI_RESID_XG) {
+                        if (interior) {
+                            if (a.f16) gemm_pp_kernel<EPI, 8, true, false, false, true, true><<<grid_tp, 512, LDS_BYTES, s>>>(ar, tiles_m, tiles_n);
+                            else gemm_pp_kernel<EPI, 8, false, false, false, true, true><<<grid_tp, 512, LDS_BYTES, s>>>(ar, tiles_m, tiles_n);
+                            HIPTS_LAUNCH_CHECK();
+                            return HIPTS_OK;
+                        }
+                    }
+                    if (a.f16) gemm_pp_kernel<EPI, 8, true, false, false, false, true><<<grid_tp, 512, LDS_BYTES, s>>>(ar, tiles_m, tiles_n);
+                    else gemm_pp_kernel<EPI, 8, false, false, false, false, true><<<grid_tp, 512, LDS_BYTES, s>>>(ar, tiles_m, tiles_n);
+                    HIPTS_LAUNCH_CHECK();
+                    return HIPTS_OK;
+                }
+            }
+            (void)pieces;
             if constexpr (EPI == EPI_RESID_XG) {
-                if (mr == 8 && a.M % 256 == 0 && a.N % 256 == 0 && a.N <= 1024 && !a.pos && !a.res_scale && a.out_bf16 && a.stat_part && !resid_general) {
+                if (mr == 8 && a.M % 256 == 0 && a.N % 256 == 0 && a.N <= 1024 && !a.pos && !a.res_scale && a.out_bf16 && a.stat_part && !resid_general && !a.resid_general) {
                     static PerDevice attr_int;
                     {
                         std::lock_guard<std::mutex> lk(attr_int.mu);
@@ -1159,6 +1276,9 @@
 }
 
 void set_gemm_q4_mask(unsigned mask) { g_q4_mask.store((long long)mask, std::memory_order_relaxed); }
+void set_gemm_tail_pieces(int on) { g_tail_pieces.store(on < 0 ? -2 : (on != 0 ? 1 : 0), std::memory_order_relaxed); }
+void set_gemm_slots(int slots) { g_slots_override.store(slots > 0 ? slots : 0, std::memory_order_relaxed); }
+int gemm_last_items() { return g_last_items; }
 
 namespace {
 __global__ void gelu_probe_kernel(const f32x4* __restrict__ x, f32x4* __restrict__ y, int n4, int tanh_form) {
diff --git a/anime-illust-image-searcher_amd/csrc/gemm_epi.h b/anime-illust-image-searcher_amd/csrc/gemm_epi.h
--- a/anime-illust-image-searcher_amd/csrc/gemm_epi.h
+++ b/anime-illust-image-searcher_amd/csrc/gemm_epi.h
@@ -504,12 +504,12 @@
             char* image = scratch + (wave_m * 4 + wave_n) * 4096;
             float2* red = reinterpret_cast<float2*>(scratch + 8 * 4096);
             if constexpr (INT) {
-                static_assert(MR == 8, "interior epilogue: full tiles");
+                static_assert(MR == 8 || MR == 4, "interior epilogue: full tiles and their 128-row halves");
                 const f32x4* cvec = colvec + (ncol0 >> 2);
                 const int lane_off = a.x_blocked ? lr * 16 + 4 * lq : lr * ld + 4 * lq;
                 const size_t rb_step = a.x_blocked ? (size_t)(ld >> 4) * 256 : (size_t)16 * ld;
                 const int cb_step = a.x_blocked ? 256 : 16;
-                float* base = a.out_f32 + x_off(a, m0 + wave_m * 128, ncol0, ld);
+                float* base = a.out_f32 + x_off(a, m0 + wave_m * (MR * 16), ncol0, ld);
                 constexpr int DEPTH = HIPTS_INT_DEPTH;
                 f32x4 xv[DEPTH][RB][4];
                 auto request = [&](int buf, int i2) {
@@ -522,19 +522,19 @@
                 request(0, 0);
                 if constexpr (DEPTH == 3) request(1, RB);
 #pragma unroll
-                for (int i2 = 0; i2 < 8; i2 += RB) {
+                for (int i2 = 0; i2 < MR; i2 += RB) {
                     epi_turn(a, wave_m, i2 / RB);
                     const int cur = (i2 / RB) % DEPTH;
                     if constexpr (DEPTH == 3) {
-                        if (i2 + 2 * RB < 8) request((cur + 2) % 3, i2 + 2 * RB);
+                        if (i2 + 2 * RB < MR) request((cur + 2) % 3, i2 + 2 * RB);
                     } else {
-                        if (i2 + RB < 8) request(cur ^ 1, i2 + RB);
+                        if (i2 + RB < MR) request(cur ^ 1, i2 + RB);
                     }
                     __builtin_amdgcn_sched_barrier(0);
 #pragma unroll
                     for (int u = 0; u < RB; ++u) {
                         float2 st = make_float2(1.f, 0.f);
-                        if constexpr (fold) st = st_lds ? st_lds[wave_m * 128 + (i2 + u) * 16 + lr] : row_stat(a, m0 + wave_m * 128 + (i2 + u) * 16 + lr);
+                        if constexpr (fold) st = st_lds ? st_lds[wave_m * (MR * 16) + (i2 + u) * 16 + lr] : row_stat(a, m0 + wave_m * (MR * 16) + (i2 + u) * 16 + lr);
 #pragma unroll
                         for (int j = 0; j < 4; ++j) {
                             const f32x4 bj = cvec[256 + j * 4 + lq];
@@ -555,9 +555,9 @@
                         float s1 = (t[0] + t[1]) + (t[2] + t[3]), s2 = (q[0] + q[1]) + (q[2] + q[3]);
                         s1 += __shfl_xor(s1, 16); s2 += __shfl_xor(s2, 16);
                         s1 += __shfl_xor(s1, 32); s2 += __shfl_xor(s2, 32);
-                        if (lq == 0) red[(wave_m * 128 + i * 16 + lr) * 4 + wave_n] = make_float2(s1, s2);
-                    }
-                    staged_store_2blocks_interior<F16>(image, lane, a.out_bf16 + (size_t)(m0 + wave_m * 128 + i2 * 16) * ld + ncol0, ld,
+                        if (lq == 0) red[(wave_m * (MR * 16) + i * 16 + lr) * 4 + wave_n] = make_float2(s1, s2);
+                    }
+                    staged_store_2blocks_interior<F16>(image, lane, a.out_bf16 + (size_t)(m0 + wave_m * (MR * 16) + i2 * 16) * ld + ncol0, ld,
                                                        [&](int u, int j) { return acc[i2 + u][j] * cvec[j * 4 + lq]; });
                     __builtin_amdgcn_sched_barrier(0);
                 }
diff --git a/anime-illust-image-searcher_amd/csrc/vit.hip b/anime-illust-image-searcher_amd/csrc/vit.hip
--- a/anime-illust-image-searcher_amd/csrc/vit.hip
+++ b/anime-illust-image-searcher_amd/csrc/vit.hip
@@ -1029,6 +1029,82 @@
     return HIPTS_OK;
 }
 
+extern "C" int hiptsdbg_gemm_set_tail_pieces(int on) {
+    set_gemm_tail_pieces(on);
+    return HIPTS_OK;
+}
+
+extern "C" int hiptsdbg_gemm_set_slots(int slots) {
+    HIPTS_REQUIRE(slots >= 0 && slots <= 4096, "hiptsdbg_gemm_set_slots: 0 .. 4096");
+    set_gemm_slots(slots);
+    return HIPTS_OK;
+}
+
+extern "C" int hiptsdbg_gemm_resid_run(int M, int N, int K, int epi, int f16, int general, float* x_host, uint16_t* copy_host, float* stat_host,
+                                       int* items_out, int iters, float* us_out) {
+    HIPTS_TRY(use_device(0));
+    HIPTS_REQUIRE((epi == EPI_RESID || epi == EPI_RESID_XG) && M >= 1 && N >= 16 && N % 16 == 0 && K >= 64 && K % 64 == 0 && (iters == 0 || us_out),
+                  "hiptsdbg_gemm_resid_run: unsupported launch");
+    const int Np = round_up(N, 256);
+    DevBuf A, W, bias, gamma, of32, obf, statp;
+    HIPTS_TRY(A.alloc((size_t)M * K * 2));
+    HIPTS_TRY(W.alloc((size_t)Np * K * 2));
+    HIPTS_TRY(bias.alloc((size_t)Np * 4));
+    HIPTS_TRY(gamma.alloc((size_t)Np * 4));
+    HIPTS_TRY(of32.alloc((size_t)M * N * 4));
+    HIPTS_TRY(obf.alloc((size_t)M * N * 2));
+    HIPTS_TRY(statp.alloc((size_t)(Np / 256) * M * 8));
+    {
+        std::vector<uint16_t> ha((size_t)M * K), hw((size_t)Np * K, 0);
+        std::vector<float> hb((size_t)Np, 0.f), hg((size_t)Np, 0.f), hx((size_t)M * N);
+        uint32_t st = 97531u + (uint32_t)(M + 3 * N + 7 * K);
+        auto rnd = [&]() { st = st * 1664525u + 1013904223u; return ((st >> 8) & 0xffff) / 65536.0f * 2.0f - 1.0f; };
+        for (auto& v : ha) v = f16 ? f32_to_f16_rne(rnd()) : f32_to_bf16_rne(rnd());
+        for (size_t i = 0; i < (size_t)N * K; ++i) hw[i] = f16 ? f32_to_f16_rne(rnd() * 0.05f) : f32_to_bf16_rne(rnd() * 0.05f);
+        for (int i = 0; i < N; ++i) hb[i] = rnd() * 0.3f;
+        for (int i = 0; i < N; ++i) hg[i] = 1.0f + rnd() * 0.2f;
+        for (auto& v : hx) v = rnd() * 3.0f;
+        HIPTS_TRY(upload(A.p, ha.data(), ha.size() * 2));
+        HIPTS_TRY(upload(W.p, hw.data(), hw.size() * 2));
+        HIPTS_TRY(upload(bias.p, hb.data(), hb.size() * 4));
+        HIPTS_TRY(upload(gamma.p, hg.data(), hg.size() * 4));
+        HIPTS_TRY(upload(of32.p, hx.data(), hx.size() * 4));
+    }
+    HIPTS_HIP(hipMemset(obf.p, 0, obf.bytes));
+    HIPTS_HIP(hipMemset(statp.p, 0, statp.bytes));
+    GemmArgs g{};
+    g.A = A.as<bf16_t>(); g.W = W.as<bf16_t>(); g.M = M; g.N = N; g.K = K; g.bias = bias.as<float>(); g.f16 = f16 ? 1 : 0;
+    g.out_f32 = of32.as<float>();
+    if (epi == EPI_RESID_XG) {
+        g.out_bf16 = obf.as<bf16_t>(); g.ln_gamma = gamma.as<float>(); g.stat_part = statp.as<float>(); g.stat_stride = M;
+        g.resid_general = general ? 1 : 0;
+    }
+    g.shared_chip = 1;
+    HIPTS_TRY(launch_gemm((GemmEpilogue)epi, g, nullptr));
+    if (items_out) *items_out = gemm_last_items();
+    HIPTS_HIP(hipDeviceSynchronize());
+    if (x_host) HIPTS_HIP(hipMemcpy(x_host, of32.p, of32.bytes, hipMemcpyDeviceToHost));
+    if (copy_host) HIPTS_HIP(hipMemcpy(copy_host, obf.p, obf.bytes, hipMemcpyDeviceToHost));
+    if (stat_host) HIPTS_HIP(hipMemcpy(stat_host, statp.p, statp.bytes, hipMemcpyDeviceToHost));
+    if (iters > 0) {
+        hipEvent_t e0, e1;
+        HIPTS_HIP(hipEventCreate(&e0));
+        HIPTS_HIP(hipEventCreate(&e1));
+        for (int i = 0; i < iters; ++i) {
+            HIPTS_HIP(hipEventRecord(e0, nullptr));
+            HIPTS_TRY(launch_gemm((GemmEpilogue)epi, g, nullptr));
+            HIPTS_HIP(hipEventRecord(e1, nullptr));
+            HIPTS_HIP(hipEventSynchronize(e1));
+            float ms = 0.f;
+            HIPTS_HIP(hipEventElapsedTime(&ms, e0, e1));
+            us_out[i] = ms * 1000.f;
+        }
+        (void)hipEventDestroy(e0);
+        (void)hipEventDestroy(e1);
+    }
+    return HIPTS_OK;
+}
+
 extern "C" int hiptsdbg_gemm_run(int M, int N, int K, const uint16_t* a_bf16, const uint16_t* w_bf16, float* out_host) {
     HIPTS_TRY(use_device(0));
     HIPTS_REQUIRE(M >= 1 && N >= 16 && N % 16 == 0 && K >= 64 && K % 64 == 0, "hiptsdbg_gemm_run: unsupported shape");
diff --git a/anime-illust-image-searcher_amd/csrc/vit_internal.h b/anime-illust-image-searcher_amd/csrc/vit_internal.h
--- a/anime-illust-image-searcher_amd/csrc/vit_internal.h
+++ b/anime-illust-image-searcher_amd/csrc/vit_internal.h
@@ -227,6 +227,8 @@
     void* sk_ws = nullptr;
     size_t sk_ws_bytes = 0;
     int sk_first = 0, sk_slices = 1;
+    int tp_first = 0;
+    int resid_general = 0;
     int raster_gn = 0;
     int raster_gm = 0;
     int x_blocked = 0;
@@ -242,6 +244,9 @@
 int launch_gemm_q4(GemmEpilogue epi, const GemmArgs& a, hipStream_t s, bool* handled);
 constexpr unsigned GEMM_Q4_DEFAULT_MASK = 0u;
 void set_gemm_q4_mask(unsigned mask);
+void set_gemm_tail_pieces(int on);
+void set_gemm_slots(int slots);
+int gemm_last_items();
 long long gemm_q4_launch_count();
 constexpr size_t GEMM_SK_WS_BYTES = 4096 + 256 * (size_t)(256 * 256 * 4);
 
diff --git a/include/hip_tagsearch_debug.h b/include/hip_tagsearch_debug.h
--- a/include/hip_tagsearch_debug.h
+++ b/include/hip_tagsearch_debug.h
@@ -13,6 +13,10 @@
 int hiptsdbg_gemm_time(int M, int N, int K, int epi, int iters, float* ms_out);
 int hiptsdbg_gemm_clock(int M, int N, int K, int epi, int iters, float* ms_out, float* loop_ghz);
 int hiptsdbg_gemm_q4_compare(int M, int N, int K, int epi, int f16, int iters, long long* mismatch_out, float* ms_out);
+int hiptsdbg_gemm_set_tail_pieces(int on);
+int hiptsdbg_gemm_set_slots(int slots);
+int hiptsdbg_gemm_resid_run(int M, int N, int K, int epi, int f16, int general, float* x_host, uint16_t* copy_host, float* stat_host,
+                            int* items_out, int iters, float* us_out);
 int hiptsdbg_gelu(const float* x_host, int n, int tanh_form, float* y_host);
 int hiptsdbg_dwconv7(const uint16_t* in_f16, const float* w, uint16_t* out_f16, int batch, int H, int C, int mode, int iters, float* ms_out);
 int hiptsdbg_dwconv7_stamps(unsigned long long* host, int n);
```

After: 4792 images/sec. 11.7% lower.
